# grero/HMMSpikeSorter.jl

Measured on AMD Instinct MI355X. Metric: Msamples/sec (Viterbi + forward-backward), K=4 L=60 HMM, higher is better.
Workload: dtype f64; 1 GPU; K=4 L=60 HMM (reference N=4, K=60: 237 states), 10000000-sample single channel per GPU: one Viterbi decode + one Baum-Welch E-step (forward-backward + sufficient statistics + M-step finish); channels=1, samples_per_channel=10000000, states=237, engine=wave, block=4928, halo=295, chains=2030, seed=1234, pooled_allreduce=False

## Files before the change

### hmmspikesorter.jl_amd/csrc/capi.cpp

```cpp
#include <algorithm>
#include <cstring>
#include <memory>

#include "hmmsort_internal.h"

using namespace hmmsort;

int hmmsort::need_device()
{
    int n = 0;
    hipError_t e = hipGetDeviceCount(&n);
    if (e != hipSuccess || n < 1) {
        (void)hipGetLastError();
        set_error("no HIP device available (%s); libhmmsort_hip has no CPU fallback",
                  e == hipSuccess ? "device count is 0" : hipGetErrorString(e));
        return HMMSORT_EHIP;
    }
    return HMMSORT_OK;
}

int hmmsort::plan_create_engine(hmmsort_plan **out, int64_t T, const int16_t *states, int64_t N, int64_t K,
                                int64_t S, const hmm_trans *tr, int64_t R, const double *mu, double sigma,
                                int64_t engine_req, int64_t halo_req)
{
    HS_CHECK(out, HMMSORT_EINVAL, "plan_create: null output pointer");
    *out = nullptr;
    HS_CHECK(T >= 1, HMMSORT_EINVAL, "plan_create: T must be >= 1 (got %lld)", (long long)T);
    int rc = need_device();
    if (rc) return rc;
    const Options opt = options_get();
    std::unique_ptr<hmmsort_plan> p(new hmmsort_plan());
    p->T = T;
    rc = build_host_model(p->model, states, N, K, S, tr, R, mu, sigma);
    if (rc) return rc;
    std::string why;
    const bool wave_ok = wave_supported(p->model, T, &why);
    if (engine_req == HMMSORT_ENGINE_WAVE && !wave_ok) {
        set_error("wave engine unavailable for this model/signal: %s", why.c_str());
        return HMMSORT_EUNSUP;
    }
    const bool ring_ok = ring_supported(p->model, T, &why);
    if (engine_req == HMMSORT_ENGINE_RING && !ring_ok) {
        set_error("ring engine unavailable for this model/signal: %s", why.c_str());
        return HMMSORT_EUNSUP;
    }
    const bool want_ring = engine_req == HMMSORT_ENGINE_RING;
    const int64_t halo = halo_req >= 0 ? halo_req : opt.halo;
    if ((engine_req == HMMSORT_ENGINE_AUTO || engine_req == HMMSORT_ENGINE_WAVE) && wave_ok) {
        p->models.assign(1, p->model);
        rc = wave_engine_create(&p->eng, p->models, T, opt.block, halo);
    } else if (want_ring && ring_ok) {
        rc = ring_engine_create(&p->eng, p->model, T, opt.block, halo);
    } else if (engine_req == HMMSORT_ENGINE_BLOCKED ||
               (engine_req == HMMSORT_ENGINE_AUTO && T >= blocked_min_samples())) {
        rc = generic_engine_create(&p->eng, p->model, T, true, opt.block, halo, opt.blocked_hbm_columns);
        if (rc == HMMSORT_EUNSUP && engine_req == HMMSORT_ENGINE_AUTO) rc = generic_engine_create(&p->eng, p->model, T);
    } else {
        rc = generic_engine_create(&p->eng, p->model, T);
    }
    if (rc) return rc;
    *out = p.release();
    return HMMSORT_OK;
}

extern "C" {

const char *hmmsort_last_error(void) { return last_error(); }
int hmmsort_version(void) { return 110;  }

int hmmsort_device_count(int *count)
{
    HS_CHECK(count, HMMSORT_EINVAL, "device_count: null pointer");
    int n = 0;
    if (hipGetDeviceCount(&n) != hipSuccess) {
        (void)hipGetLastError();
        n = 0;
    }
    *count = n;
    return HMMSORT_OK;
}

int hmmsort_set_device(int device)
{
    HS_HIP(hipSetDevice(device));
    return HMMSORT_OK;
}

int hmmsort_set_option(const char *key, int64_t value)
{
    HS_CHECK(key, HMMSORT_EINVAL, "set_option: null key");
    if (!strcmp(key, "engine")) {
        HS_CHECK(value >= 0 && value <= 4, HMMSORT_EINVAL, "set_option: engine must be 0..4");
        options_modify([&](Options &o) { o.engine = value; });
    } else if (!strcmp(key, "block")) {
        HS_CHECK(value >= 0, HMMSORT_EINVAL, "set_option: block must be >= 0");
        options_modify([&](Options &o) { o.block = value; });
    } else if (!strcmp(key, "halo")) {
        HS_CHECK(value >= 0, HMMSORT_EINVAL, "set_option: halo must be >= 0");
        options_modify([&](Options &o) { o.halo = value; });
    } else if (!strcmp(key, "escalate")) {
        options_modify([&](Options &o) { o.escalate = value != 0; });
    } else if (!strcmp(key, "strict_limit_mb")) {
        HS_CHECK(value >= 0, HMMSORT_EINVAL, "set_option: strict_limit_mb must be >= 0");
        options_modify([&](Options &o) { o.strict_limit_mb = value; });
    } else if (!strcmp(key, "blocked_hbm_columns")) {
        HS_CHECK(value >= 0 && value <= 2, HMMSORT_EINVAL, "set_option: blocked_hbm_columns must be 0..2");
        options_modify([&](Options &o) { o.blocked_hbm_columns = value; });
    } else if (!strcmp(key, "tie_scale")) {
        HS_CHECK(value >= 1, HMMSORT_EINVAL, "set_option: tie_scale must be >= 1");
        options_modify([&](Options &o) { o.tie_scale = value; });
    } else if (!strcmp(key, "tie_debug")) {
        HS_CHECK(value >= 0 && value <= 3, HMMSORT_EINVAL, "set_option: tie_debug must be 0..3");
        options_modify([&](Options &o) { o.tie_debug = value; });
    } else if (!strcmp(key, "backtrace")) {
        HS_CHECK(value >= 0 && value <= 2, HMMSORT_EINVAL, "set_option: backtrace must be 0..2");
        options_modify([&](Options &o) { o.backtrace = value; });
    } else if (!strcmp(key, "fit_streams")) {
        HS_CHECK(value >= 1 && value <= 16, HMMSORT_EINVAL, "set_option: fit_streams must be 1..16");
        options_modify([&](Options &o) { o.fit_streams = value; });
    } else if (!strcmp(key, "plan_cache")) {
        HS_CHECK(value >= 0 && value <= 64, HMMSORT_EINVAL, "set_option: plan_cache must be 0..64");
        options_modify([&](Options &o) { o.plan_cache = value; });
        host_slots_trim((size_t)value);
    } else {
        set_error("set_option: unknown key '%s'", key);
        return HMMSORT_EINVAL;
    }
    return HMMSORT_OK;
}

int hmmsort_get_option(const char *key, int64_t *value)
{
    HS_CHECK(key && value, HMMSORT_EINVAL, "get_option: null argument");
    const Options o = options_get();
    if (!strcmp(key, "engine")) *value = o.engine;
    else if (!strcmp(key, "block")) *value = o.block;
    else if (!strcmp(key, "halo")) *value = o.halo;
    else if (!strcmp(key, "escalate")) *value = o.escalate;
    else if (!strcmp(key, "plan_cache")) *value = o.plan_cache;
    else if (!strcmp(key, "strict_limit_mb")) *value = o.strict_limit_mb;
    else if (!strcmp(key, "blocked_hbm_columns")) *value = o.blocked_hbm_columns;
    else if (!strcmp(key, "tie_scale")) *value = o.tie_scale;
    else if (!strcmp(key, "tie_debug")) *value = o.tie_debug;
    else if (!strcmp(key, "backtrace")) *value = o.backtrace;
    else if (!strcmp(key, "fit_streams")) *value = o.fit_streams;
    else if (!strcmp(key, "last_escalations")) *value = last_escalations();
    else {
        set_error("get_option: unknown key '%s'", key);
        return HMMSORT_EINVAL;
    }
    return HMMSORT_OK;
}

int hmmsort_shutdown(void)
{
    host_slots_trim(0);
    return HMMSORT_OK;
}


int hmmsort_plan_create(hmmsort_plan **plan_out, int64_t T, const int16_t *states, int64_t N,
                        int64_t K, int64_t S, const hmm_trans *tr, int64_t R, const double *mu,
                        double sigma)
{
    return plan_create_engine(plan_out, T, states, N, K, S, tr, R, mu, sigma, options_get().engine);
}

int hmmsort_plan_create_batched(hmmsort_plan **plan_out, int64_t C, int64_t T, const int16_t *states,
                                int64_t N, int64_t K, int64_t S, const hmm_trans *tr, int64_t R,
                                const double *mu, const double *sigma)
{
    HS_CHECK(plan_out, HMMSORT_EINVAL, "plan_create_batched: null output pointer");
    *plan_out = nullptr;
    HS_CHECK(C >= 1 && C <= 4096 && T >= 1 && tr && mu && sigma, HMMSORT_EINVAL,
             "plan_create_batched: bad argument (C = %lld, T = %lld)", (long long)C, (long long)T);
    int rc = need_device();
    if (rc) return rc;
    std::unique_ptr<hmmsort_plan> p(new hmmsort_plan());
    p->T = T;
    p->C = C;
    p->models.resize(C);
    for (int64_t ch = 0; ch < C; ch++) {
        rc = build_host_model(p->models[ch], states, N, K, S, tr + ch * R, R, mu + ch * K * N, sigma[ch]);
        if (rc) return rc;
    }
    p->model = p->models[0];
    std::string why;
    if (!wave_supported(p->model, T, &why)) {
        set_error("plan_create_batched needs the wave engine: %s", why.c_str());
        return HMMSORT_EUNSUP;
    }
    const Options opt = options_get();
    rc = wave_engine_create(&p->eng, p->models, T, opt.block, opt.halo);
    if (rc) return rc;
    *plan_out = p.release();
    return HMMSORT_OK;
}

int64_t hmmsort_plan_channels(const hmmsort_plan *p) { return p ? p->C : 0; }

static int plan_set_model(const char *who, hmmsort_plan *p, int64_t channel, const hmm_trans *tr, int64_t R,
                          const double *mu, double sigma)
{
    HostModel m;
    std::vector<int16_t> st = p->model.states;
    int rc = build_host_model(m, st.data(), p->model.N, p->model.K, p->model.S, tr, R, mu, sigma);
    if (rc) return rc;
    HS_CHECK(!p->eng->ring_models_only() || m.ring.valid, HMMSORT_EUNSUP, "%s: new model is not a ring model", who);
    if ((rc = p->eng->set_model(channel, m))) return rc;
    if (!p->models.empty()) p->models[channel] = m;
    if (channel == 0) p->model = std::move(m);
    p->pu_stale = true;
    return HMMSORT_OK;
}

int hmmsort_plan_set_model_channel(hmmsort_plan *p, int64_t channel, const hmm_trans *tr, int64_t R,
                                   const double *mu, double sigma)
{
    HS_CHECK(p && tr && mu, HMMSORT_EINVAL, "plan_set_model_channel: null argument");
    HS_CHECK(p->eng->id == HMMSORT_ENGINE_WAVE, HMMSORT_EUNSUP, "plan_set_model_channel: needs a wave-engine plan");
    HS_CHECK(channel >= 0 && channel < p->C, HMMSORT_EINVAL, "plan_set_model_channel: channel %lld outside 0..%lld",
             (long long)channel, (long long)p->C - 1);
    return plan_set_model("plan_set_model_channel", p, channel, tr, R, mu, sigma);
}

int hmmsort_plan_set_model(hmmsort_plan *p, const hmm_trans *tr, int64_t R, const double *mu,
                           double sigma)
{
    HS_CHECK(p && tr && mu, HMMSORT_EINVAL, "plan_set_model: null argument");
    HS_CHECK(R == p->model.R || p->eng->ring_models_only(), HMMSORT_EINVAL,
             "plan_set_model: R changed (%lld -> %lld)", (long long)p->model.R, (long long)R);
    return plan_set_model("plan_set_model", p, 0, tr, R, mu, sigma);
}

int hmmsort_plan_destroy(hmmsort_plan *p)
{
    delete p;
    return HMMSORT_OK;
}

int hmmsort_plan_info(const hmmsort_plan *p, int64_t *engine, int64_t *block, int64_t *halo,
                      int64_t *nchains, int64_t *workspace_bytes)
{
    HS_CHECK(p, HMMSORT_EINVAL, "plan_info: null plan");
    int64_t b = 0, h = 0, n = 0;
    p->eng->geometry(&b, &h, &n);
    if (engine) *engine = p->eng->id;
    if (block) *block = b;
    if (halo) *halo = h;
    if (nchains) *nchains = n;
    if (workspace_bytes) *workspace_bytes = p->eng->workspace_bytes();
    return HMMSORT_OK;
}

int64_t hmmsort_plan_overlap_sweep(const hmmsort_plan *p) { return p ? p->eng->overlap_sweep() : 0; }

int hmmsort_plan_bind(hmmsort_plan *p, const double *d_y, void *stream)
{
    HS_CHECK(p && d_y, HMMSORT_EINVAL, "plan_bind: null argument");
    return p->eng->bind(d_y, (hipStream_t)stream);
}

int hmmsort_plan_unbind(hmmsort_plan *p)
{
    HS_CHECK(p, HMMSORT_EINVAL, "plan_unbind: null plan");
    p->eng->unbind();
    return HMMSORT_OK;
}

int hmmsort_plan_viterbi(hmmsort_plan *p, const double *d_y, int16_t *d_x, double *d_ll,
                         void *stream)
{
    HS_CHECK(p && d_y && d_x && d_ll, HMMSORT_EINVAL, "plan_viterbi: null argument");
    return p->eng->viterbi(d_y, d_x, d_ll, (hipStream_t)stream);
}

int hmmsort_plan_decode_estep(hmmsort_plan *p, const double *d_y, int16_t *d_x, double *d_ll,
                              double *d_stats, void *stream)
{
    HS_CHECK(p && d_y && d_x && d_ll && d_stats, HMMSORT_EINVAL, "plan_decode_estep: null argument");
    return p->eng->decode_estep(d_y, d_x, d_ll, d_stats, (hipStream_t)stream);
}

int hmmsort_plan_set_shard(hmmsort_plan *p, int64_t own_lo, int64_t own_hi, int first, int last)
{
    HS_CHECK(p, HMMSORT_EINVAL, "plan_set_shard: null plan");
    int rc = p->eng->set_shard(own_lo, own_hi, first != 0, last != 0);
    if (rc == HMMSORT_OK) p->sharded = !(own_lo == 0 && own_hi == p->T && first && last);
    return rc;
}

int64_t hmmsort_plan_stats_len(const hmmsort_plan *p) { return p ? p->eng->stats_len() : 0; }

int64_t hmmsort_plan_mstep_len(const hmmsort_plan *p)
{
    if (!p) return 0;
    const HostModel &m = p->model;
    return m.K * m.N + 1 + p->eng->n_lp() + m.S;
}

int hmmsort_plan_estep(hmmsort_plan *p, const double *d_y, double *d_stats, void *stream)
{
    HS_CHECK(p && d_y && d_stats, HMMSORT_EINVAL, "plan_estep: null argument");
    return p->eng->estep(d_y, d_stats, (hipStream_t)stream);
}

int hmmsort_plan_mstep(hmmsort_plan *p, const double *d_stats, double *d_out, void *stream)
{
    HS_CHECK(p && d_stats && d_out, HMMSORT_EINVAL, "plan_mstep: null argument");
    return p->eng->mstep(d_stats, d_out, (hipStream_t)stream);
}

int hmmsort_plan_path_update(hmmsort_plan *p, const double *d_y, const int16_t *d_x, double *d_out,
                             int64_t *d_counts, void *stream)
{
    HS_CHECK(p && d_y && d_x && d_out, HMMSORT_EINVAL, "plan_path_update: null argument");
    HS_CHECK(!p->sharded, HMMSORT_EINVAL, "plan_path_update: the plan is a time shard (hmmsort_plan_set_shard); the "
                                          "update needs the whole recording");
    return plan_path_update(p, d_y, d_x, d_out, d_counts, (hipStream_t)stream);
}

int hmmsort_plan_diagnostics(hmmsort_plan *p, void *stream, int64_t diag[8])
{
    HS_CHECK(p && diag, HMMSORT_EINVAL, "plan_diagnostics: null argument");
    for (int i = 0; i < 8; i++) diag[i] = 0;
    return p->eng->diagnostics((hipStream_t)stream, diag);
}

int hmmsort_plan_tie_stats(hmmsort_plan *p, void *stream, int64_t out[8])
{
    HS_CHECK(p && out, HMMSORT_EINVAL, "plan_tie_stats: null argument");
    for (int i = 0; i < 8; i++) out[i] = 0;
    return p->eng->tie_stats((hipStream_t)stream, out);
}

int hmmsort_plan_debug_record(hmmsort_plan *p, double *out64)
{
    HS_CHECK(p && out64, HMMSORT_EINVAL, "plan_debug_record: needs a wave plan");
    return p->eng->debug_record(out64);
}

int hmmsort_plan_debug_array(hmmsort_plan *p, int which, double *out, int64_t n)
{
    HS_CHECK(p && out, HMMSORT_EINVAL, "plan_debug_array: needs a wave plan");
    return p->eng->debug_array(which, out, n);
}

int hmmsort_plan_profile(hmmsort_plan *p, int enable)
{
    HS_CHECK(p, HMMSORT_EINVAL, "plan_profile: null plan");
    return p->eng->profile(enable);
}

int hmmsort_plan_profile_read(hmmsort_plan *p, void *stream, char *names, int64_t names_cap,
                              double *ms, int64_t *calls, int64_t cap, int64_t *n_out)
{
    HS_CHECK(p && names && ms && calls && n_out, HMMSORT_EINVAL, "plan_profile_read: null argument");
    *n_out = 0;
    if (names_cap > 0) names[0] = 0;
    std::vector<std::string> nm;
    std::vector<double> m;
    std::vector<int64_t> c;
    int rc = p->eng->profile_read((hipStream_t)stream, nm, m, c);
    if (rc) return rc;
    std::string joined;
    int64_t n = std::min<int64_t>((int64_t)nm.size(), cap);
    for (int64_t i = 0; i < n; i++) {
        if (i) joined += "\n";
        joined += nm[i];
        ms[i] = m[i];
        calls[i] = c[i];
    }
    HS_CHECK((int64_t)joined.size() + 1 <= names_cap, HMMSORT_EINVAL, "plan_profile_read: names buffer too small");
    memcpy(names, joined.c_str(), joined.size() + 1);
    *n_out = n;
    return HMMSORT_OK;
}

int hmmsort_samples_to_f64(const void *d_in, int sample_type, int64_t T, int64_t stride, double *d_out,
                           void *stream)
{
    HS_CHECK(T >= 0 && stride >= 1 && (T == 0 || (d_in && d_out)), HMMSORT_EINVAL,
             "samples_to_f64: bad argument (T = %lld, stride = %lld)", (long long)T, (long long)stride);
    int rc = need_device();
    if (rc) return rc;
    return dev_widen(d_in, sample_type, T, stride, d_out, (hipStream_t)stream);
}

int hmmsort_reconstruct(const int16_t *x, int64_t T, const int16_t *states, int64_t N, int64_t S,
                        const double *mu, int64_t K, double *y_out)
{
    HS_CHECK(states && mu && (T == 0 || (x && y_out)), HMMSORT_EINVAL, "reconstruct: null argument");
    HS_CHECK(T >= 0 && N >= 1 && S >= 1 && K >= 1, HMMSORT_EINVAL, "reconstruct: bad sizes");
    if (T == 0) return HMMSORT_OK;
    int rc = need_device();
    if (rc) return rc;
    for (int64_t i = 0; i < T; i++)
        HS_CHECK(x[i] >= 1 && x[i] <= S, HMMSORT_EINVAL,
                 "reconstruct: x[%lld] = %d outside 1..S (reference would throw BoundsError)",
                 (long long)i, (int)x[i]);
    DevBuf dx, dst, dmu, dout;
    if ((rc = dx.alloc(T * sizeof(int16_t))) || (rc = dst.alloc(N * S * sizeof(int16_t))) ||
        (rc = dmu.alloc(K * N * sizeof(double))) || (rc = dout.alloc(T * sizeof(double))))
        return rc;
    HS_HIP(hipMemcpy(dx.p, x, T * sizeof(int16_t), hipMemcpyHostToDevice));
    HS_HIP(hipMemcpy(dst.p, states, N * S * sizeof(int16_t), hipMemcpyHostToDevice));
    HS_HIP(hipMemcpy(dmu.p, mu, K * N * sizeof(double), hipMemcpyHostToDevice));
    rc = dev_reconstruct(dx.as<int16_t>(), T, dst.as<int16_t>(), N, S, dmu.as<double>(), K,
                         dout.as<double>(), nullptr);
    if (rc) return rc;
    HS_HIP(hipDeviceSynchronize());
    HS_HIP(hipMemcpy(y_out, dout.p, T * sizeof(double), hipMemcpyDeviceToHost));
    return HMMSORT_OK;
}

int hmmsort_unroll_mlseq(const int16_t *mlseq, int64_t T, const int16_t *states, int64_t N,
                         int64_t S, int16_t *out)
{
    HS_CHECK(states && (T == 0 || (mlseq && out)), HMMSORT_EINVAL, "unroll_mlseq: null argument");
    if (T == 0) return HMMSORT_OK;
    int rc = need_device();
    if (rc) return rc;
    for (int64_t i = 0; i < T; i++)
        HS_CHECK(mlseq[i] >= 1 && mlseq[i] <= S, HMMSORT_EINVAL,
                 "unroll_mlseq: mlseq[%lld] = %d outside 1..S", (long long)i, (int)mlseq[i]);
    DevBuf dx, dst, dout;
    if ((rc = dx.alloc(T * sizeof(int16_t))) || (rc = dst.alloc(N * S * sizeof(int16_t))) ||
        (rc = dout.alloc((size_t)N * T * sizeof(int16_t))))
        return rc;
    HS_HIP(hipMemcpy(dx.p, mlseq, T * sizeof(int16_t), hipMemcpyHostToDevice));
    HS_HIP(hipMemcpy(dst.p, states, N * S * sizeof(int16_t), hipMemcpyHostToDevice));
    rc = dev_unroll(dx.as<int16_t>(), T, dst.as<int16_t>(), N, S, dout.as<int16_t>(), nullptr);
    if (rc) return rc;
    HS_HIP(hipDeviceSynchronize());
    HS_HIP(hipMemcpy(out, dout.p, (size_t)N * T * sizeof(int16_t), hipMemcpyDeviceToHost));
    return HMMSORT_OK;
}

static int extract_from_device(const int16_t *d_x, int64_t T, const int16_t *states, int64_t N,
                               int64_t S, const double *mu, int64_t K, int64_t *times_out,
                               int64_t cap, int64_t *counts_out, hipStream_t st, DevBuf *dt_keep = nullptr)
{
    std::vector<uint32_t> match(S, 0u);
    for (int64_t i = 0; i < N; i++) {
        const int32_t qv = trough_value(mu, K, i);
        for (int64_t j = 0; j < S; j++)
// ... 153 lines not shown
```

### hmmspikesorter.jl_amd/csrc/hmmsort_internal.h

```cpp
#pragma once
#include <hip/hip_runtime.h>
#include <stdint.h>
#include <functional>
#include <memory>
#include <string>
#include <vector>
#include "../../include/hmmsort.h"

namespace hmmsort {

void set_error(const char *fmt, ...);
const char *last_error();

#define HS_HIP(call)                                                                          \
    do {                                                                                      \
        hipError_t e_ = (call);                                                               \
        if (e_ != hipSuccess) {                                                               \
            hmmsort::set_error("%s failed: %s (%s:%d)", #call, hipGetErrorString(e_),         \
                               __FILE__, __LINE__);                                           \
            return HMMSORT_EHIP;                                                              \
        }                                                                                     \
    } while (0)

#define HS_CHECK(cond, code, ...)                                                             \
    do {                                                                                      \
        if (!(cond)) {                                                                        \
            hmmsort::set_error(__VA_ARGS__);                                                  \
            return (code);                                                                    \
        }                                                                                     \
    } while (0)

constexpr double kLog2Pi = 0.9189385332046727;

struct Options {
    int64_t engine = HMMSORT_ENGINE_AUTO;
    int64_t block = 0;
    int64_t halo = 0;
    int64_t escalate = 1;
    int64_t plan_cache = 4;
    int64_t strict_limit_mb = 0;
    int64_t tie_scale = 1;
    int64_t blocked_hbm_columns = 0;
    int64_t tie_debug = 0;
    int64_t fit_streams = 4;
    int64_t backtrace = 0;
};
Options options_get();
void options_modify(const std::function<void(Options &)> &f);
int64_t &last_escalations();

struct RingModel {
    bool valid = false;
    int N = 0, L = 0;
    double c00 = 0;
    std::vector<double> c0;
    std::vector<double> cint;
    std::vector<double> cend;
    std::vector<double> cx;
};

struct HostModel {
    int64_t N = 0, K = 0, S = 0, R = 0;
    std::vector<int16_t> states;
    std::vector<hmm_trans> tr;
    std::vector<double> mu;
    double sigma = 0;
    std::vector<double> mean;
    std::vector<int32_t> in_ptr, in_src;
    std::vector<double> in_lp;
    std::vector<int32_t> out_ptr, out_dst;
    std::vector<double> out_lp;
    RingModel ring;
};

int build_host_model(HostModel &m, const int16_t *states, int64_t N, int64_t K, int64_t S,
                     const hmm_trans *tr, int64_t R, const double *mu, double sigma);
int analyze_ring(const HostModel &m, RingModel &ring);
inline int32_t trough_value(const double *mu, int64_t K, int64_t i)
{
    int64_t q = 0;
    for (int64_t k = 1; k < K; k++)
        if (mu[k + K * i] < mu[q + K * i]) q = k;
    return (int32_t)(q + 1);
}
inline double strict_limit_bytes(const Options &opt)
{
    size_t free_b = 0, total_b = 0;
    if (hipMemGetInfo(&free_b, &total_b) != hipSuccess) { (void)hipGetLastError(); free_b = 0; }
    return opt.strict_limit_mb > 0 ? (double)opt.strict_limit_mb * 1048576.0 : 0.9 * (double)free_b;
}

struct DevBuf {
    void *p = nullptr;
    size_t cap = 0;
    ~DevBuf() { release(); }
    void release()
    {
        if (p) (void)hipFree(p);
        p = nullptr;
        cap = 0;
    }
    int alloc(size_t bytes)
    {
        release();
        bytes = bytes < 8 ? 8 : bytes;
        if (hipMalloc(&p, bytes) != hipSuccess) {
            (void)hipGetLastError();
            set_error("hipMalloc of %zu bytes failed", bytes);
            p = nullptr;
            return HMMSORT_ENOMEM;
        }
        cap = bytes;
        return HMMSORT_OK;
    }
    int ensure(size_t bytes) { return (p && cap >= (bytes < 8 ? 8 : bytes)) ? HMMSORT_OK : alloc(bytes); }
    template <typename Tv> Tv *as() { return static_cast<Tv *>(p); }
};

class Engine {
public:
    const int64_t id;
    explicit Engine(int64_t id_) : id(id_) {}
    virtual ~Engine() = default;
    Engine(const Engine &) = delete;
    Engine &operator=(const Engine &) = delete;

    virtual int set_model(int64_t channel, const HostModel &m) = 0;
    virtual bool ring_models_only() const { return false; }
    virtual void geometry(int64_t *block, int64_t *halo, int64_t *nchains) const = 0;
    virtual int64_t workspace_bytes() const = 0;
    virtual int bind(const double *, hipStream_t) { return HMMSORT_OK; }
    virtual void unbind() {}
    virtual int viterbi(const double *d_y, int16_t *d_x, double *d_ll, hipStream_t st) = 0;
    virtual int decode_estep(const double *, int16_t *, double *, double *, hipStream_t)
    {
        return refuse(HMMSORT_EUNSUP, "plan_decode_estep: needs the wave or ring engine");
    }
    virtual int64_t stats_len() const { return 0; }
    bool has_estep() const { return stats_len() > 0; }
    virtual int estep(const double *, double *, hipStream_t)
    {
        return refuse(HMMSORT_EUNSUP, "plan_estep: sufficient-statistics E-step needs the wave, ring or blocked "
                                      "engine (use hmmsort_em_step)");
    }
    virtual int mstep(const double *, double *, hipStream_t)
    {
        return refuse(HMMSORT_EUNSUP, "plan_mstep: needs the wave, ring or blocked engine");
    }
    virtual int64_t n_lp() const = 0;
    virtual int set_shard(int64_t, int64_t, bool, bool)
    {
        return refuse(HMMSORT_EUNSUP, "plan_set_shard: needs the wave or ring engine");
    }
    virtual int diagnostics(hipStream_t, int64_t[8]) { return HMMSORT_OK; }
    virtual int tie_stats(hipStream_t, int64_t[8]) { return HMMSORT_OK; }
    virtual int profile(int) { return HMMSORT_OK; }
    virtual int profile_read(hipStream_t, std::vector<std::string> &, std::vector<double> &, std::vector<int64_t> &)
    {
        return HMMSORT_OK;
    }
    virtual bool has_posteriors() const { return false; }
    virtual int posteriors(const HostModel &, const double *, double *, double *, double *, double *, hipStream_t)
    {
        set_error("plan_posteriors: needs a wave plan (ring models), a blocked plan (overlap models within the LDS "
                  "limit) or a strict plan (any model); this plan runs engine %lld", (long long)id);
        return HMMSORT_EUNSUP;
    }
    virtual bool posteriors_valid() const { return false; }
    virtual int posterior_decode(int16_t *, hipStream_t)
    {
        return refuse(HMMSORT_EINVAL, "plan_posterior_decode: call hmmsort_plan_posteriors first");
    }
    virtual int spike_conf(int, int, int, int64_t, const int64_t *, int64_t, double *, hipStream_t)
    {
        return refuse(HMMSORT_EINVAL, "plan_spike_confidence: call hmmsort_plan_posteriors first");
    }
    virtual int expected_counts(double *, hipStream_t)
    {
        return refuse(HMMSORT_EINVAL, "plan_expected_counts: call hmmsort_plan_posteriors first");
    }
    virtual int64_t overlap_sweep() const { return 0; }
    virtual bool drop_structured_sweep() { return false; }
    virtual int forward(const double *, double *, hipStream_t) { return refuse(HMMSORT_EUNSUP, "forward: needs the strict engine"); }
    virtual int backward(const double *, double *, hipStream_t) { return refuse(HMMSORT_EUNSUP, "backward: needs the strict engine"); }
    virtual int update(const double *, const double *, const double *, double *, hipStream_t)
    {
        return refuse(HMMSORT_EUNSUP, "update: needs the strict engine");
    }
    virtual int debug_record(double *) { return refuse(HMMSORT_EINVAL, "plan_debug_record: needs a wave plan"); }
    virtual int debug_array(int, double *, int64_t) { return refuse(HMMSORT_EINVAL, "plan_debug_array: needs a wave plan"); }

protected:
    static int refuse(int code, const char *msg)
    {
        set_error("%s", msg);
        return code;
    }
    static int check_shard(int64_t T, int64_t own_lo, int64_t own_hi, bool first, bool last)
    {
        HS_CHECK(own_lo >= 0 && own_lo <= own_hi && own_hi <= T, HMMSORT_EINVAL,
                 "plan_set_shard: owned range [%lld, %lld) outside [0, %lld]", (long long)own_lo,
                 (long long)own_hi, (long long)T);
        HS_CHECK((!first || own_lo == 0) && (!last || own_hi == T), HMMSORT_EINVAL,
                 "plan_set_shard: a first/last shard must own its first/last sample");
        return HMMSORT_OK;
    }
};

bool wave_supported(const HostModel &m, int64_t T, std::string *why);
int wave_engine_create(std::unique_ptr<Engine> *out, const std::vector<HostModel> &models, int64_t T,
                       int64_t block_req, int64_t halo_req);
int ring_engine_create(std::unique_ptr<Engine> *out, const HostModel &m, int64_t T, int64_t block_req,
                       int64_t halo_req);
int generic_engine_create(std::unique_ptr<Engine> *out, const HostModel &m, int64_t T, bool blocked = false,
                          int64_t block_req = 0, int64_t halo_req = 0, int64_t hbm_columns = 0);

struct GenericDev;
struct RingDev;
struct PathUpdateDev;

int generic_create(GenericDev **g, const HostModel &m, int64_t T, bool blocked = false,
                   int64_t block_req = 0, int64_t halo_req = 0);
bool generic_pair_active(const GenericDev *g);
void generic_pair_disable(GenericDev *g);
int64_t generic_overlap_sweep(const GenericDev *g);
int64_t blocked_min_samples();
int generic_set_model(GenericDev *g, const HostModel &m);
void generic_destroy(GenericDev *g);
int generic_viterbi(GenericDev *g, const double *d_y, int16_t *d_x, double *d_ll,
                    hipStream_t st);
int generic_forward(GenericDev *g, const double *d_y, double *d_alpha, hipStream_t st);
int generic_backward(GenericDev *g, const double *d_y, double *d_beta, hipStream_t st);
int generic_update(GenericDev *g, const double *d_alpha, const double *d_beta, const double *d_y,
                   double *d_out, hipStream_t st);
int generic_posteriors(const double *d_alpha, const double *d_beta, int64_t T, int64_t S, int64_t N,
                       const int16_t *d_states, const int32_t *d_qv, double *d_logz, double *d_onset,
                       double *d_occ, double *d_silent, double *d_tq, int16_t *d_xm, hipStream_t st);
bool blocked_estep_supported(const GenericDev *g);
void blocked_set_hbm_columns(GenericDev *g, int64_t v);
bool blocked_post_supported(const GenericDev *g);
int blocked_posteriors(GenericDev *g, const double *d_y, const int32_t *trough, double *d_onset, double *d_occ,
                       double *d_silent, double *d_tq, int16_t *d_xm, double *d_logz, hipStream_t st);

int ring_create(RingDev **r, const HostModel &m, int64_t T, int64_t block_req, int64_t halo_req);
int ring_set_model(RingDev *r, const HostModel &m);
void ring_destroy(RingDev *r);
int ring_diagnostics(RingDev *r, hipStream_t st, int64_t diag[8]);
bool ring_supported(const HostModel &m, int64_t T, std::string *why);

int dev_reconstruct(const int16_t *d_x, int64_t T, const int16_t *d_states, int64_t N, int64_t S,
                    const double *d_mu, int64_t K, double *d_out, hipStream_t st);
int dev_widen(const void *d_in, int dtype, int64_t T, int64_t stride, double *d_out, hipStream_t st);
constexpr int kSpikeChunkHost = 4096;
int dev_spike_compact(const int16_t *d_x, int64_t T, const uint32_t *d_match, int N, int S, int pass,
                      int64_t *d_cnt, const int64_t *d_offs, int64_t *d_times, int64_t cap,
                      hipStream_t st);
int dev_unroll(const int16_t *d_x, int64_t T, const int16_t *d_states, int64_t N, int64_t S,
               int16_t *d_out, hipStream_t st);
int dev_chunk_stitch(const int16_t *d_x, int64_t k, bool lead, bool trail, int16_t *d_dst, int64_t *d_lk,
                     hipStream_t st);
int dev_fill_i16(int16_t *d_p, int64_t n, int16_t v, hipStream_t st);
int dev_chunk_ll(const double *d_y, const int16_t *d_x, int64_t k, int64_t S, const double *d_mean,
                 const int32_t *d_in_ptr, const int32_t *d_in_src, const double *d_in_lp, double sigma, double *d_pv,
                 double *d_ll, hipStream_t st);
constexpr int kPostParts = 256;
int dev_spike_conf(const double *d_src, const double *d_head, int64_t T, int64_t shift, int64_t jitter,
                   const int64_t *d_times, int64_t n, double *d_conf, hipStream_t st);
int dev_row_sums(const double *d_rows, int64_t nrows, int64_t T, double *d_part, double *out_host, hipStream_t st);

}

struct hmmsort_plan {
    hmmsort::HostModel model;
    std::vector<hmmsort::HostModel> models;
    int64_t T = 0;
    int64_t C = 1;
    std::unique_ptr<hmmsort::Engine> eng;
    bool sharded = false;
    std::shared_ptr<hmmsort::PathUpdateDev> pu;
    bool pu_stale = true;
};

namespace hmmsort {
int need_device();
int plan_create_engine(hmmsort_plan **out, int64_t T, const int16_t *states, int64_t N, int64_t K, int64_t S,
                       const hmm_trans *tr, int64_t R, const double *mu, double sigma, int64_t engine_req,
                       int64_t halo_req = -1);
struct PlanGuard {
    hmmsort_plan *p = nullptr;
    ~PlanGuard() { if (p) hmmsort_plan_destroy(p); }
};
int plan_path_update(hmmsort_plan *p, const double *d_y, const int16_t *d_x, double *d_out, int64_t *d_counts,
                     hipStream_t st);
void host_slots_trim(size_t keep);
}
```

### hmmspikesorter.jl_amd/csrc/wave_common.h

```cpp
#pragma once
#include <hip/hip_runtime.h>
#include <stdint.h>
#include <cmath>
#include <cstring>
#include <string>
#include <vector>

#include "hmmsort_internal.h"
#include "ring_common.h"

namespace hmmsort {

constexpr double kScFloor = -700.0;

struct WaveGeom {
    int64_t T;
    int C;
    int N, L;
    int W;
    int RB;
    int B;
    int Hw;
    int He;
    int nch;
    int EB, epw, PW;
    int Bb, Hb;
    int64_t nseg;
    int64_t own_lo, own_hi;
    int first, last;
    double thr_scale;
    int tie_debug;
    int backtrace;
};

struct WaveConst {
    double c00, mean0, den, A, sc0, P00;
    double c0[kRingMaxN], cend[kRingMaxN], sc[kRingMaxN], CP0[kRingMaxN], PEND[kRingMaxN];
    double xishift[kRingMaxN];
    double cx[kRingMaxN * kRingMaxN];
    double CPX[kRingMaxN * kRingMaxN];
    double cxin[kRingMaxN];
    double CPXin[kRingMaxN];
    double cxT[kRingMaxN * kRingMaxN];
    double CPXT[kRingMaxN * kRingMaxN];
};

struct WaveDev {
    WaveGeom g{};
    bool prof_on = false;
    bool uniform_cx = true;
    std::vector<char> ucx;
    const double *bound_y = nullptr;
    hipStream_t side = nullptr, side2 = nullptr;
    hipEvent_t ev_fork = nullptr, ev_join = nullptr, ev_a = nullptr, ev_b = nullptr, ev_c = nullptr, ev_x = nullptr;
    std::vector<ProfEntry> prof;
    int64_t S = 0, K = 0;
    std::vector<RingModel> ring;
    std::vector<std::vector<double>> mean;
    std::vector<double> sigma;
    WaveConst *d_cst = nullptr;
    double *d_mean = nullptr;
    double *d_meanT = nullptr;
    double *d_msq = nullptr;
    double *d_cint = nullptr;
    double *d_ctab = nullptr;
    int16_t *d_states = nullptr;
    double *Rf = nullptr;
    double *W2 = nullptr;
    double *virt = nullptr;
    double *ysum = nullptr;
    uint32_t *psi = nullptr;
    double *vpre = nullptr, *vend = nullptr;
    int32_t *vfail = nullptr;
    int32_t *bstate = nullptr;
    int32_t *redo = nullptr;
    int32_t *final_state = nullptr;
    double *part = nullptr;
    double *FA0 = nullptr;
    double *FV = nullptr;
    double *FREF = nullptr;
    double *fpre = nullptr;
    double *bpre = nullptr, *bown = nullptr;
    double *rho = nullptr;
    double *Zc = nullptr;
    double *partS = nullptr;
    double *partG = nullptr;
    double *yhead = nullptr;
    double *extra = nullptr;
    double *pp = nullptr;
    int64_t *diag = nullptr;
    int32_t *heads = nullptr;
    int32_t *vlist = nullptr;
    double *trash = nullptr;
    double *dbg = nullptr;
    bool keep_post = false;
    bool post_valid = false;
    double *gsil = nullptr;
    double *phead = nullptr;
    double *plogz = nullptr;
    double *pcnt = nullptr;
    int64_t *tie_cnt = nullptr;
    int64_t *tie_list = nullptr;
    int64_t *tie_off = nullptr;
    int64_t tie_ntile = 0;
    int16_t *tie_walk = nullptr;
    double *tie_guess = nullptr;
    double *tie_c = nullptr;
    int32_t *tie_ok = nullptr;
    double *tie_v = nullptr;
    int64_t tie_nblk = 0;
    struct GraphEntry { uint64_t key[12]; hipGraphExec_t exec; };
    std::vector<GraphEntry> graphs;
    bool graphs_on = true;
    int64_t bytes = 0;
    int nparts = 0, gparts = 0;
};

struct WProfScope {
    WaveDev *r;
    hipStream_t st;
    ProfEntry e;
    WProfScope(WaveDev *r_, const char *name, hipStream_t st_) : r(r_), st(st_)
    {
        e.name = name; e.a = nullptr; e.b = nullptr;
        if (r->prof_on && hipEventCreate(&e.a) == hipSuccess && hipEventCreate(&e.b) == hipSuccess)
            (void)hipEventRecord(e.a, st);
    }
    ~WProfScope()
    {
        if (r->prof_on && e.a && e.b) {
            (void)hipEventRecord(e.b, st);
            r->prof.push_back(e);
        }
    }
};
#define WPROF(r, name, st) WProfScope wprof_scope_(r, name, st)

constexpr int wpsi_bits_c(int N) { int b = 1; while ((1 << b) < N + 1) b++; return b + 1; }
constexpr int wpsi_epw_c(int N) { return 32 / wpsi_bits_c(N); }
constexpr int wpsi_words_c(int N) { return (N + 1 + wpsi_epw_c(N) - 1) / wpsi_epw_c(N); }

__device__ __forceinline__ double wave_bcast(double v, int lane)
{
    const int lo = __builtin_amdgcn_readlane(__double2loint(v), lane);
    const int hi = __builtin_amdgcn_readlane(__double2hiint(v), lane);
    return __hiloint2double(hi, lo);
}

template <int CTRL, int ROWMASK>
__device__ __forceinline__ double dpp_mov(double old, double v)
{
    const int lo = __builtin_amdgcn_update_dpp(__double2loint(old), __double2loint(v), CTRL, ROWMASK, 0xF, false);
    const int hi = __builtin_amdgcn_update_dpp(__double2hiint(old), __double2hiint(v), CTRL, ROWMASK, 0xF, false);
    return __hiloint2double(hi, lo);
}

__device__ __forceinline__ double lane_prev(double v, double carry)
{
    return dpp_mov<0x138, 0xF>(carry, v);
}

__device__ __forceinline__ void scan_maxplus(double &a, double &b)
{
#define HS_MP_STEP(CTRL, RM)                                                      \
    {                                                                             \
        const double al = dpp_mov<CTRL, RM>(0.0, a), bl = dpp_mov<CTRL, RM>(-INFINITY, b); \
        b = fmax(bl + a, b);                                                      \
        a = al + a;                                                               \
    }
    HS_MP_STEP(0x111, 0xF) HS_MP_STEP(0x112, 0xF) HS_MP_STEP(0x114, 0xF) HS_MP_STEP(0x118, 0xF)
    HS_MP_STEP(0x142, 0xA) HS_MP_STEP(0x143, 0xC)
#undef HS_MP_STEP
}

template <int CTRL, int ROWMASK>
__device__ __forceinline__ float dpp_movf(float old, float v)
{
    return __int_as_float(__builtin_amdgcn_update_dpp(__float_as_int(old), __float_as_int(v), CTRL, ROWMASK, 0xF, false));
}
__device__ __forceinline__ void scan_maxplus_f32(float &a, float &b)
{
#define HS_MPF_STEP(CTRL, RM)                                                     \
    {                                                                             \
        const float al = dpp_movf<CTRL, RM>(0.0f, a), bl = dpp_movf<CTRL, RM>(-INFINITY, b); \
        b = fmaxf(bl + a, b);                                                     \
        a = al + a;                                                               \
    }
    HS_MPF_STEP(0x111, 0xF) HS_MPF_STEP(0x112, 0xF) HS_MPF_STEP(0x114, 0xF) HS_MPF_STEP(0x118, 0xF)
    HS_MPF_STEP(0x142, 0xA) HS_MPF_STEP(0x143, 0xC)
#undef HS_MPF_STEP
}
__device__ __forceinline__ float lane_prevf(float v, float carry)
{
    return dpp_movf<0x138, 0xF>(carry, v);
}

__device__ __forceinline__ void scan_linear(double &a, double &b)
{
#define HS_LN_STEP(CTRL, RM)                                                      \
    {                                                                             \
        const double al = dpp_mov<CTRL, RM>(1.0, a), bl = dpp_mov<CTRL, RM>(0.0, b); \
        b = __builtin_fma(a, bl, b);                                              \
        a = al * a;                                                               \
    }
    HS_LN_STEP(0x111, 0xF) HS_LN_STEP(0x112, 0xF) HS_LN_STEP(0x114, 0xF) HS_LN_STEP(0x118, 0xF)
    HS_LN_STEP(0x142, 0xA) HS_LN_STEP(0x143, 0xC)
#undef HS_LN_STEP
}

__device__ __forceinline__ double lane_prev_ref(double v, double carry, int lane)
{
    const double s = __shfl_up(v, 1);
    return lane == 0 ? carry : s;
}
__device__ __forceinline__ void scan_maxplus_ref(double &a, double &b, int lane)
{
#pragma unroll
    for (int d = 1; d < 64; d <<= 1) {
        const double al = __shfl_up(a, d), bl = __shfl_up(b, d);
        if (lane >= d) { b = fmax(bl + a, b); a = al + a; }
    }
}
__device__ __forceinline__ void scan_linear_ref(double &a, double &b, int lane)
{
#pragma unroll
    for (int d = 1; d < 64; d <<= 1) {
        const double al = __shfl_up(a, d), bl = __shfl_up(b, d);
        if (lane >= d) { b = __builtin_fma(a, bl, b); a = al * a; }
    }
}

__device__ __forceinline__ const WaveConst *reload_consts(const WaveConst *p)
{
    asm volatile("" : "+s"(p));
    return p;
}

template <int N> constexpr int wave_depth() { return N <= 4 ? 4 : (N <= 8 ? 3 : 2); }
template <int N> constexpr int wave_occ() { return N <= 4 ? 4 : (N <= 8 ? 2 : 1); }

__device__ __forceinline__ double wave_max(double v)
{
#pragma unroll
    for (int o = 32; o > 0; o >>= 1) v = fmax(v, __shfl_xor(v, o));
    return v;
}
__device__ __forceinline__ double wave_sum(double v)
{
#pragma unroll
    for (int o = 32; o > 0; o >>= 1) v += __shfl_xor(v, o);
    return v;
}

__device__ __forceinline__ void wave_lds_order()
{
    __builtin_amdgcn_fence(__ATOMIC_RELEASE, "wavefront");
    __builtin_amdgcn_wave_barrier();
    __builtin_amdgcn_fence(__ATOMIC_ACQUIRE, "wavefront");
}

constexpr int kTieBlk = 512;
constexpr int kTieCap = 65536;
constexpr int kTieWalk = 8192;
constexpr int kTieLanes = 64;
constexpr int kTieTrig = 0;
constexpr int kTieListed = 1;
constexpr int kTieDone = 2;
constexpr int kTieFlips = 3;
constexpr int kTieOpen = 4;
constexpr int kTieTail = 5;
constexpr int kTieLongest = 6;
constexpr int kTieSerial = 7;

__device__ __forceinline__ double wpath_lp(int N, int L, const double *__restrict__ ctab, int xp, int xc)
{
    if (xp == 1) return xc == 1 ? ctab[0] : ctab[1 + (xc - 2) / L];
    const int a = (xp - 2) / L, k = (xp - 2) % L + 1;
    if (k < L) return ctab[1 + 2 * N + N * N + a * L + k];
    if (xc == 1) return ctab[1 + N + a];
    return ctab[1 + 2 * N + a * N + (xc - 2) / L];
}

__device__ __forceinline__ double wave_thr(const WaveGeom &g, const WaveConst &K, const double *__restrict__ ysum, int ch)
{
    const double T = (double)g.T;
    const double s1 = ysum[2 * ch], s2 = ysum[2 * ch + 1];
    const double sq = fmax((s2 - 2.0 * K.mean0 * s1) + T * K.mean0 * K.mean0, 0.0);
    const double mmax = fabs(K.A) * T + sq / K.den + fabs(K.c00) * T + 1.0;
    return (ldexp(16.0 * (double)(g.L + 2), ilogb(mmax) - 52) + 4.0e-9) * g.thr_scale;
}

template <typename F>
int wave_graphed(WaveDev *r, int kind, const void *p0, const void *p1, const void *p2, const void *p3,
                 hipStream_t st, F enqueue)
{
    if (!r->graphs_on || r->prof_on || st == nullptr) return enqueue(st);
    uint64_t key[12] = {(uint64_t)kind, (uint64_t)(uintptr_t)p0, (uint64_t)(uintptr_t)p1, (uint64_t)(uintptr_t)p2,
                        (uint64_t)(uintptr_t)p3, (uint64_t)(uintptr_t)st, (uint64_t)(r->bound_y == p0),
                        (uint64_t)r->uniform_cx, (uint64_t)r->g.own_lo, (uint64_t)r->g.own_hi,
                        (uint64_t)(r->g.first * 2 + r->g.last), (uint64_t)(uint32_t)r->g.tie_debug};
    {
        uint64_t tb;
        static_assert(sizeof(tb) == sizeof(r->g.thr_scale), "");
        memcpy(&tb, &r->g.thr_scale, sizeof(tb));
        key[11] ^= tb << 8;
    }
    for (auto &e : r->graphs)
        if (!memcmp(e.key, key, sizeof(key))) {
            HS_HIP(hipGraphLaunch(e.exec, st));
            return HMMSORT_OK;
        }
    if (hipStreamBeginCapture(st, hipStreamCaptureModeRelaxed) != hipSuccess) {
        (void)hipGetLastError();
        r->graphs_on = false;
        return enqueue(st);
    }
    const int rc = enqueue(st);
    hipGraph_t graph = nullptr;
    const hipError_t e1 = hipStreamEndCapture(st, &graph);
    hipGraphExec_t exec = nullptr;
    if (rc || e1 != hipSuccess || !graph || hipGraphInstantiate(&exec, graph, nullptr, nullptr, 0) != hipSuccess) {
        (void)hipGetLastError();
        if (graph) (void)hipGraphDestroy(graph);
        r->graphs_on = false;
        return rc ? rc : enqueue(st);
    }
    (void)hipGraphDestroy(graph);
    if (r->graphs.size() >= 16) {
        (void)hipGraphExecDestroy(r->graphs.front().exec);
        r->graphs.erase(r->graphs.begin());
    }
    WaveDev::GraphEntry ge;
    memcpy(ge.key, key, sizeof(key));
    ge.exec = exec;
    r->graphs.push_back(ge);
    HS_HIP(hipGraphLaunch(exec, st));
    return HMMSORT_OK;
}

inline size_t wave_zero_bytes(const WaveDev *r, bool decode)
{
    return (size_t)(decode ? 8 + 8 * (int64_t)r->g.C + 2 : 8) * sizeof(int64_t);
}

int wave_create(WaveDev **out, const std::vector<HostModel> &models, int64_t T, int64_t block_req,
                int64_t halo_req);
int wave_set_model(WaveDev *r, int ch, const HostModel &m);
void wave_destroy(WaveDev *r);
int wave_prepare(WaveDev *r, const double *d_y, hipStream_t st);
int wave_bind(WaveDev *r, const double *d_y, hipStream_t st);
int64_t wave_stats_len(const WaveDev *r);
int wave_diagnostics(WaveDev *r, hipStream_t st, int64_t diag[8]);
int wave_profile_read(WaveDev *r, hipStream_t st, std::vector<std::string> &names,
                      std::vector<double> &ms, std::vector<int64_t> &calls);
int wave_viterbi_sweep(WaveDev *r, const double *d_y, hipStream_t st);
int wave_viterbi_post(WaveDev *r, const double *d_y, int16_t *d_x, double *d_ll, hipStream_t st, bool beside,
                      bool ll_beside, hipStream_t ll_st);
int wave_viterbi(WaveDev *r, const double *d_y, int16_t *d_x, double *d_ll, hipStream_t st);
int wave_tie_resolve(WaveDev *r, const double *d_y, int16_t *d_x, hipStream_t st);
int wave_tie_stats(WaveDev *r, hipStream_t st, int64_t out[8]);
int wave_estep(WaveDev *r, const double *d_y, double *d_stats, hipStream_t st);
int wave_mstep(WaveDev *r, const double *d_stats, double *d_out, hipStream_t st);
int wave_decode_estep(WaveDev *r, const double *d_y, int16_t *d_x, double *d_ll, double *d_stats,
                      hipStream_t st);
int wave_post_sweeps(WaveDev *r, const double *d_y, hipStream_t st);
int wave_posteriors(WaveDev *r, const double *d_y, double *d_onset, double *d_occ, double *d_silent, double *d_logz,
                    hipStream_t st);
int wave_post_decode(WaveDev *r, int16_t *d_xm, hipStream_t st);
int wave_spike_conf(WaveDev *r, int ch, int a, int qv, int64_t jitter, const int64_t *d_times, int64_t n,
                    double *d_conf, hipStream_t st);
int wave_expected_counts(WaveDev *r, double *counts_out, hipStream_t st);

}
```

### hmmspikesorter.jl_amd/csrc/wave_engine.hip

```cpp
#include <algorithm>
#include <cmath>
#include <cstdlib>
#include <cstring>
#include <type_traits>

#include "wave_common.h"

namespace hmmsort {

static inline int64_t wround_up(int64_t v, int64_t m) { return (v + m - 1) / m * m; }

constexpr int64_t kWaveLdsMax = 160 * 1024;

static bool ring_uniform_cx(const RingModel &R)
{
    const int N = R.N;
    for (int a = 0; a < N; a++) {
        double ref = 0.0;
        bool have = false;
        for (int b = 0; b < N; b++) {
            if (b == a) continue;
            const double v = R.cx[b * N + a];
            if (!have) { ref = v; have = true; }
            else if (!(v == ref)) return false;
        }
    }
    return true;
}

constexpr int kWaveMaxPerSource = 8;

bool wave_supported(const HostModel &m, int64_t T, std::string *why)
{
    auto no = [&](const char *w) { if (why) *why = w; return false; };
    if (!m.ring.valid) return no("transition list is not the no-overlap ring pattern");
    if (m.ring.N > kRingMaxN) return no("more than 16 rings");
    if (m.ring.N > kWaveMaxPerSource && !ring_uniform_cx(m.ring))
        return no("exit->entry log-probabilities depend on the source ring and there are more than 8 rings");
    if (m.ring.L < 8) return no("rings shorter than 8 states");
    if (T < 4 * (int64_t)m.ring.L || T < 512) return no("signal shorter than 4 ring lengths / 512 samples");
    const int W = std::min(m.ring.L, 64);
    const int64_t RB = wround_up(m.ring.L + W, 32);
    const int64_t lines = m.ring.N > 8 ? m.ring.N + 1 : 2 * (int64_t)m.ring.N;
    if (lines * (RB + 1) * 8 + 4096 > kWaveLdsMax) return no("delay lines exceed the LDS of one CU");
    return true;
}

static int make_geometry(WaveGeom &g, int64_t T, int C, int N, int L, int64_t block_req, int64_t halo_req)
{
    g.T = T; g.C = C; g.N = N; g.L = L;
    g.own_lo = 0; g.own_hi = T; g.first = 1; g.last = 1;
    { const Options o = options_get(); g.thr_scale = (double)o.tie_scale; g.tie_debug = (int)o.tie_debug;
      g.backtrace = (int)o.backtrace; }
    g.W = std::min(L, 64);
    g.RB = (int)wround_up(L + g.W, 32);
    int64_t H = halo_req > 0 ? halo_req : std::max<int64_t>(256, 4 * (int64_t)L);
    H = std::max<int64_t>(H, L + 8);
    const int64_t m = (H + g.W - 1) / g.W;
    g.Hw = (int)(1 + m * g.W);
    g.He = (int)(m * g.W);
    int64_t B = block_req > 0 ? block_req : (T * C + 2047) / 2048;
    B = std::max<int64_t>(B, std::max<int64_t>(2 * g.Hw, 512));
    if (block_req > 0) B = std::max<int64_t>(block_req, std::max<int64_t>(g.Hw, L + 16));
    B = wround_up(B, 64);
    if (B > T) B = wround_up(T, 64);
    for (;;) {
        const int64_t nch = (T + B - 1) / B;
        const int64_t nlast = T - (nch - 1) * B;
        if (nch == 1 || nlast >= L) break;
        B += 64;
    }
    HS_CHECK(B < (1 << 30), HMMSORT_EINVAL, "wave engine: chain too long");
    g.B = (int)B;
    g.nch = (int)((T + B - 1) / B);
    int bits = 1;
    while ((1 << bits) < N + 1) bits++;
    g.EB = bits + 1; g.epw = 32 / g.EB; g.PW = (N + 1 + g.epw - 1) / g.epw;
    g.Bb = 512; g.Hb = 128;
    while (g.Hb < 2 * L + 64) g.Hb += 64;
    if (g.Bb < 2 * g.Hb) g.Bb = 2 * g.Hb;
    g.nseg = (T + g.Bb - 1) / g.Bb;
    return HMMSORT_OK;
}

template <typename Tv>
static int wmalloc(Tv **p, int64_t n, int64_t *bytes)
{
    if (hipMalloc((void **)p, (size_t)std::max<int64_t>(n, 1) * sizeof(Tv)) != hipSuccess) {
        (void)hipGetLastError();
        set_error("wave engine: hipMalloc of %.2f GB failed", n * sizeof(Tv) / 1e9);
        *p = nullptr;
        return HMMSORT_ENOMEM;
    }
    *bytes += n * (int64_t)sizeof(Tv);
    return HMMSORT_OK;
}

int wave_set_model(WaveDev *r, int ch, const HostModel &m)
{
    const WaveGeom &g = r->g;
    HS_CHECK(ch >= 0 && ch < g.C, HMMSORT_EINVAL, "wave set_model: channel %d outside 0..%d", ch, g.C - 1);
    HS_CHECK(m.ring.valid && m.ring.N == g.N && m.ring.L == g.L && m.S == r->S, HMMSORT_EINVAL,
             "wave set_model: model shape changed");
    HS_CHECK(g.N <= kWaveMaxPerSource || ring_uniform_cx(m.ring), HMMSORT_EUNSUP,
             "wave set_model: exit->entry log-probabilities depend on the source ring and there are more than 8 rings");
    r->bound_y = nullptr;
    r->ring[ch] = m.ring;
    r->mean[ch] = m.mean;
    r->sigma[ch] = m.sigma;
    const int N = g.N, L = g.L;
    const RingModel &R = m.ring;
    WaveConst k;
    memset(&k, 0, sizeof(k));
    k.c00 = R.c00;
    k.mean0 = m.mean[0];
    k.den = 2.0 * (m.sigma * m.sigma);
    k.A = -kLog2Pi - std::log(m.sigma);
    double sc0 = R.c00;
    for (int a = 0; a < N; a++) sc0 = std::max(sc0, R.cend[a]);
    if (!std::isfinite(sc0)) sc0 = 0.0;
    k.sc0 = sc0;
    k.P00 = std::exp(R.c00 - sc0);
    for (int a = 0; a < N; a++) {
        k.c0[a] = R.c0[a];
        k.cend[a] = R.cend[a];
        k.PEND[a] = std::exp(R.cend[a] - sc0);
        double sc = R.c0[a];
        for (int b = 0; b < N; b++)
            if (b != a) sc = std::max(sc, R.cx[b * N + a]);
        if (!std::isfinite(sc)) sc = 0.0;
        sc = std::max(sc, kScFloor);
        k.sc[a] = sc;
        k.CP0[a] = std::exp(R.c0[a] - sc);
        k.xishift[a] = R.c0[a] - sc;
    }
    for (int a = 0; a < N; a++)
        for (int b = 0; b < N; b++) {
            k.cx[a * N + b] = (a == b) ? -INFINITY : R.cx[a * N + b];
            k.CPX[a * N + b] = (a == b) ? 0.0 : std::exp(R.cx[a * N + b] - k.sc[b]);
            k.cxT[b * N + a] = k.cx[a * N + b];
            k.CPXT[b * N + a] = k.CPX[a * N + b];
        }
    bool ucx = true;
    for (int a = 0; a < N; a++) {
        double ref = -INFINITY;
        bool have = false;
        for (int b = 0; b < N; b++) {
            if (b == a) continue;
            const double v = R.cx[b * N + a];
            if (!have) { ref = v; have = true; }
            else if (!(v == ref)) ucx = false;
        }
        k.cxin[a] = have ? ref : -INFINITY;
        k.CPXin[a] = have ? std::exp(ref - k.sc[a]) : 0.0;
    }
    r->ucx[ch] = ucx;
    r->uniform_cx = true;
    for (char u : r->ucx) r->uniform_cx = r->uniform_cx && u;
    HS_HIP(hipMemcpy(r->d_cst + ch, &k, sizeof(k), hipMemcpyHostToDevice));
    HS_HIP(hipMemcpy(r->d_mean + (size_t)ch * m.S, m.mean.data(), m.S * sizeof(double), hipMemcpyHostToDevice));
    {
        const int Nn = m.ring.N, Ll = m.ring.L;
        std::vector<double> mt((size_t)Nn * Ll);
        for (int a = 0; a < Nn; a++)
            for (int k = 0; k < Ll; k++) mt[(size_t)k * Nn + a] = m.mean[1 + (size_t)a * Ll + k];
        HS_HIP(hipMemcpy(r->d_meanT + (size_t)ch * Nn * Ll, mt.data(), mt.size() * sizeof(double), hipMemcpyHostToDevice));
    }
    std::vector<double> cint((size_t)N * (L + 1), 0.0), msq((size_t)N * (L + 1), 0.0);
    for (int a = 0; a < N; a++) {
        double acc = 0.0, acc2 = 0.0;
        for (int kk = 2; kk <= L; kk++) {
            acc += R.cint[(size_t)a * L + (kk - 1)];
            cint[(size_t)a * (L + 1) + kk] = acc;
        }
        for (int kk = 1; kk <= L; kk++) {
            const double mv = m.mean[1 + (size_t)a * L + (kk - 1)];
            acc2 += mv * mv;
            msq[(size_t)a * (L + 1) + kk] = acc2;
        }
    }
    const size_t nt = (size_t)N * (L + 1);
    HS_HIP(hipMemcpy(r->d_cint + ch * nt, cint.data(), nt * sizeof(double), hipMemcpyHostToDevice));
    HS_HIP(hipMemcpy(r->d_msq + ch * nt, msq.data(), nt * sizeof(double), hipMemcpyHostToDevice));
    std::vector<double> ctab;
    ctab.push_back(R.c00);
    ctab.insert(ctab.end(), R.c0.begin(), R.c0.end());
    ctab.insert(ctab.end(), R.cend.begin(), R.cend.end());
    ctab.insert(ctab.end(), R.cx.begin(), R.cx.end());
    ctab.insert(ctab.end(), R.cint.begin(), R.cint.end());
    HS_HIP(hipMemcpy(r->d_ctab + (size_t)ch * ctab.size(), ctab.data(), ctab.size() * sizeof(double),
                     hipMemcpyHostToDevice));
    if (ch == 0)
        HS_HIP(hipMemcpy(r->d_states, m.states.data(), m.states.size() * sizeof(int16_t), hipMemcpyHostToDevice));
    return HMMSORT_OK;
}

int wave_create(WaveDev **out, const std::vector<HostModel> &models, int64_t T, int64_t block_req,
                int64_t halo_req)
{
    HS_CHECK(!models.empty(), HMMSORT_EINVAL, "wave engine: no model");
    const HostModel &m = models[0];
    std::string why;
    HS_CHECK(wave_supported(m, T, &why), HMMSORT_EUNSUP, "wave engine: %s", why.c_str());
    const int C = (int)models.size();
    WaveDev *r = new WaveDev();
    int rc = make_geometry(r->g, T, C, m.ring.N, m.ring.L, block_req, halo_req);
    if (rc) { delete r; return rc; }
    r->S = m.S; r->K = m.K;
    r->graphs_on = getenv("HMMSORT_GRAPHS") && atoi(getenv("HMMSORT_GRAPHS")) != 0;
    r->ring.resize(C); r->mean.resize(C); r->sigma.resize(C); r->ucx.assign(C, 1);
    const WaveGeom &g = r->g;
    const int64_t N = g.N, L = g.L, CT = (int64_t)C * T, nchT = (int64_t)C * g.nch;
    r->nparts = 1024;
    bool ok = true;
    auto A = [&](auto **p, int64_t n) { if (ok && wmalloc(p, n, &r->bytes)) ok = false; };
    A(&r->d_cst, C);
    A(&r->d_mean, C * m.S);
    A(&r->d_meanT, C * N * L);
    A(&r->d_cint, C * N * (L + 1));
    A(&r->d_msq, C * N * (L + 1));
    A(&r->d_ctab, C * (1 + 2 * N + N * N + N * L));
    A(&r->d_states, N * m.S);
    A(&r->Rf, N * CT);
    A(&r->W2, CT);
    A(&r->virt, C * N * (L + 1));
    A(&r->ysum, 2 * C);
    A(&r->psi, (int64_t)g.PW * CT);
    A(&r->vpre, nchT * (1 + N * L));
    A(&r->vend, nchT * (1 + N * L));
    A(&r->vfail, nchT + 8);
    A(&r->bstate, C * g.nseg);
    A(&r->redo, 2 * C * g.nseg + 8);
    A(&r->vlist, 2 * nchT + 8);
    A(&r->final_state, C + 8);
    A(&r->part, (int64_t)C * 4 * r->nparts);
    A(&r->FA0, CT);
    A(&r->FV, N * CT);
    A(&r->FREF, CT);
    A(&r->fpre, nchT * (1 + L * (N + 1)));
    A(&r->bpre, nchT * (1 + L * (N + 1)));
    A(&r->bown, nchT * (1 + L * (N + 1)));
    A(&r->rho, N * CT);
    A(&r->Zc, nchT);
    A(&r->partS, nchT * (3 * N + 3));
    r->gparts = (int)((T + 4095) / 4096);
    r->gparts = std::max<int>(r->gparts, g.nch);
    A(&r->partG, (int64_t)C * r->gparts * N * L);
    A(&r->yhead, C * (N * L + 2));
    A(&r->extra, C * 3 * N * L);
    A(&r->pp, C * m.S);
    A(&r->diag, 8 + 8 * (int64_t)C + 2);
    if (ok) { r->tie_cnt = r->diag + 8; r->heads = reinterpret_cast<int32_t *>(r->diag + 8 + 8 * (int64_t)C); }
    A(&r->dbg, 64);
    A(&r->trash, 64 * 64);
    r->tie_nblk = (T + kTieBlk - 1) / kTieBlk;
    A(&r->tie_list, (int64_t)C * kTieCap);
    r->tie_ntile = (T + 4095) / 4096;
    A(&r->tie_off, (int64_t)C * (r->tie_ntile + 1));
    A(&r->tie_walk, (int64_t)C * kTieLanes * kTieWalk);
    A(&r->tie_guess, (int64_t)C * r->tie_nblk);
    A(&r->tie_c, (int64_t)C * r->tie_nblk * 2);
    A(&r->tie_ok, (int64_t)C * r->tie_nblk);
    A(&r->tie_v, (int64_t)C * (r->tie_nblk + 1));
    if (!ok) { wave_destroy(r); return HMMSORT_ENOMEM; }
    if (getenv("HMMSORT_POISON")) {
        (void)hipMemset(r->Rf, 0xFF, N * CT * 8);
        (void)hipMemset(r->psi, 0xFF, (int64_t)g.PW * CT * 4);
        (void)hipMemset(r->vpre, 0xFF, nchT * (1 + N * L) * 8);
        (void)hipMemset(r->vend, 0xFF, nchT * (1 + N * L) * 8);
        (void)hipMemset(r->FA0, 0xFF, CT * 8);
        (void)hipMemset(r->FV, 0xFF, N * CT * 8);
        (void)hipMemset(r->FREF, 0xFF, CT * 8);
        (void)hipMemset(r->fpre, 0xFF, nchT * (1 + L * (N + 1)) * 8);
        (void)hipMemset(r->bpre, 0xFF, nchT * (1 + L * (N + 1)) * 8);
        (void)hipMemset(r->bown, 0xFF, nchT * (1 + L * (N + 1)) * 8);
        (void)hipMemset(r->rho, 0xFF, N * CT * 8);
        (void)hipMemset(r->Zc, 0xFF, nchT * 8);
        (void)hipMemset(r->partS, 0xFF, nchT * (3 * N + 3) * 8);
        (void)hipMemset(r->partG, 0xFF, (int64_t)C * r->gparts * N * L * 8);
        (void)hipMemset(r->yhead, 0xFF, C * (N * L + 2) * 8);
    }
    if (hipMemset(r->diag, 0, wave_zero_bytes(r, true)) != hipSuccess ||
        hipMemset(r->vfail, 0, (nchT + 8) * sizeof(int32_t)) != hipSuccess) {
        wave_destroy(r);
        return HMMSORT_EHIP;
    }
    for (int ch = 0; ch < C; ch++) {
        const HostModel &mc = models[ch];
        if (mc.S != m.S || mc.K != m.K || mc.N != m.N) {
            set_error("wave engine: channel %d has a different model shape", ch);
            wave_destroy(r);
            return HMMSORT_EINVAL;
        }
        rc = wave_set_model(r, ch, mc);
        if (rc) { wave_destroy(r); return rc; }
    }
    if (hipStreamCreateWithFlags(&r->side, hipStreamNonBlocking) != hipSuccess ||
        hipStreamCreateWithFlags(&r->side2, hipStreamNonBlocking) != hipSuccess ||
        hipEventCreateWithFlags(&r->ev_fork, hipEventDisableTiming) != hipSuccess ||
        hipEventCreateWithFlags(&r->ev_join, hipEventDisableTiming) != hipSuccess ||
        hipEventCreateWithFlags(&r->ev_a, hipEventDisableTiming) != hipSuccess ||
        hipEventCreateWithFlags(&r->ev_b, hipEventDisableTiming) != hipSuccess ||
        hipEventCreateWithFlags(&r->ev_c, hipEventDisableTiming) != hipSuccess ||
        hipEventCreateWithFlags(&r->ev_x, hipEventDisableTiming) != hipSuccess) {
        set_error("wave engine: could not create the internal stream/events");
        wave_destroy(r);
        return HMMSORT_EHIP;
    }
    *out = r;
    return HMMSORT_OK;
}

void wave_destroy(WaveDev *r)
{
    if (!r) return;
    void *ptrs[] = {r->d_cst, r->d_mean, r->d_meanT, r->d_cint, r->d_msq, r->d_ctab, r->d_states, r->Rf, r->W2, r->virt, r->ysum,
                    r->psi, r->vpre, r->vend, r->vfail, r->bstate, r->redo, r->final_state, r->part, r->FA0,
                    r->FV, r->FREF, r->fpre, r->bpre, r->bown, r->rho, r->Zc, r->partS, r->partG, r->yhead,
                    r->extra, r->pp, r->diag, r->vlist, r->dbg, r->trash, r->tie_list, r->tie_off, r->tie_walk, r->tie_guess,
                    r->tie_c, r->tie_ok, r->tie_v, r->gsil, r->phead, r->plogz, r->pcnt};
    for (void *p : ptrs)
        if (p) (void)hipFree(p);
    if (r->ev_fork) (void)hipEventDestroy(r->ev_fork);
    if (r->ev_join) (void)hipEventDestroy(r->ev_join);
    if (r->ev_a) (void)hipEventDestroy(r->ev_a);
    if (r->ev_b) (void)hipEventDestroy(r->ev_b);
    if (r->ev_c) (void)hipEventDestroy(r->ev_c);
    if (r->ev_x) (void)hipEventDestroy(r->ev_x);
    if (r->side) (void)hipStreamDestroy(r->side);
    if (r->side2) (void)hipStreamDestroy(r->side2);
    for (auto &e : r->prof) { (void)hipEventDestroy(e.a); (void)hipEventDestroy(e.b); }
    for (auto &ge : r->graphs) (void)hipGraphExecDestroy(ge.exec);
    delete r;
}

int wave_diagnostics(WaveDev *r, hipStream_t st, int64_t diag[8])
{
    HS_HIP(hipStreamSynchronize(st));
    HS_HIP(hipMemcpy(diag, r->diag, 8 * sizeof(int64_t), hipMemcpyDeviceToHost));
    return HMMSORT_OK;
}

int64_t wave_stats_len(const WaveDev *r) { return 3 * (int64_t)r->g.N * r->g.L + r->g.N + 4; }

__device__ __forceinline__ void virtual_onsets(const WaveGeom &g, int ch, const WaveConst *__restrict__ cst,
                                               const double *__restrict__ y, const double *__restrict__ mean,
                                               const double *__restrict__ cint, double *__restrict__ virt)
{
    const int L = g.L, N = g.N, S = 1 + N * L;
    const double *yc = y + (int64_t)ch * g.T, *mc = mean + (int64_t)ch * S;
    const double *ci = cint + (int64_t)ch * N * (L + 1);
    const double den = cst[ch].den, A = cst[ch].A;
    for (int i = threadIdx.x; i < N * L; i += blockDim.x) {
        const int a = i / L, j = i % L + 1;
        double v;
        if (j == L) {
            v = -INFINITY;
        } else if (j == L - 1) {
            const double d = yc[0] - mc[1 + a * L + (L - 1)];
            v = (A - (d * d) / den) - A;
        } else {
            double acc = 0.0;
            for (int k0 = 1 + j; k0 <= L; k0 += 8) {
                double yv[8], mv[8];
#pragma unroll
                for (int u = 0; u < 8; u++) {
                    const int k = k0 + u <= L ? k0 + u : L;
                    yv[u] = yc[k - 1 - j]; mv[u] = mc[1 + a * L + (k - 1)];
                }
#pragma unroll
                for (int u = 0; u < 8; u++) {
                    const double d = yv[u] - mv[u];
                    if (k0 + u <= L) acc += d * d;
                }
            }
            v = (ci[a * (L + 1) + L] - ci[a * (L + 1) + (1 + j)]) - acc / den;
        }
        virt[((int64_t)ch * N + a) * (L + 1) + j] = v;
    }
}

template <int N> constexpr int pre_rows() { return N <= 4 ? 8 : 4; }

template <int N> static size_t pre_lds(int L)
{
    constexpr int R = pre_rows<N>();
    const int n = 256 * R + (L > 256 ? L : 256);
    return (size_t)(n + n / R + 2) * sizeof(double);
}

template <int N>
__global__ __launch_bounds__(256) void kw_prepass(WaveGeom g, const WaveConst *__restrict__ cst,
                                                  const double *__restrict__ y,
                                                  const double *__restrict__ mean,
                                                  const double *__restrict__ cint,
                                                  const double *__restrict__ msq,
                                                  double *__restrict__ Rf, double *__restrict__ W2,
                                                  double *__restrict__ ysum, const double *__restrict__ mean_states,
                                                  double *__restrict__ virt)
{
    constexpr int R = pre_rows<N>(), TILE = 256 * R;
    extern __shared__ double ly[];
    __shared__ double red[8];
    const int ch = blockIdx.y, L = g.L, tid = threadIdx.x;
    if (blockIdx.x == 0) {
        virtual_onsets(g, ch, cst, y, mean_states, cint, virt);
        return;
    }
    const int64_t T = g.T, t0 = (int64_t)(blockIdx.x - 1) * TILE;
    const double *yc = y + (int64_t)ch * T;
    const double *mc = mean + (int64_t)ch * N * L;
    auto pad = [](int i) { return i + i / R; };
    double s1 = 0.0, s2 = 0.0;
    {
        const double *yt = yc + t0;
        const int nv = (int)(T - t0 < TILE + 512 ? T - t0 : TILE + 512);
        double v[R + 1];
#pragma unroll
        for (int q = 0; q <= R; q++) {
            const unsigned i = tid + 256 * q;
            v[q] = yt[i < (unsigned)nv ? i : (unsigned)nv - 1u];
        }
#pragma unroll
        for (int q = 0; q <= R; q++) {
            const int i = tid + 256 * q;
            const double yv = i < nv ? v[q] : 0.0;
            ly[pad(i)] = yv;
            if (q < R) { s1 += yv; s2 = __builtin_fma(yv, yv, s2); }
        }
        for (int i = TILE + 256 + tid; i < TILE + L; i += 256) {
            const int64_t t = t0 + i;
            const double yv = yc[t < T ? t : T - 1];
            ly[pad(i)] = t < T ? yv : 0.0;
        }
    }
    s1 = wave_sum(s1); s2 = wave_sum(s2);
    if ((tid & 63) == 0) { red[tid >> 6] = s1; red[4 + (tid >> 6)] = s2; }
    __syncthreads();
    if (tid == 0) {
        atomicAdd(&ysum[2 * ch], (red[0] + red[1]) + (red[2] + red[3]));
        atomicAdd(&ysum[2 * ch + 1], (red[4] + red[5]) + (red[6] + red[7]));
    }
    constexpr int U = R + 1;
    double dot[R][N], ysq[R], w[U];
#pragma unroll
    for (int r = 0; r < R; r++) {
        ysq[r] = 0.0;
        w[r] = ly[pad(R * tid + r)];
#pragma unroll
        for (int a = 0; a < N; a++) dot[r][a] = 0.0;
    }
    double mv[N];
#pragma unroll
    for (int a = 0; a < N; a++) mv[a] = mc[a];
    for (int k0 = 0; k0 < L; k0 += U) {
#pragma unroll
        for (int kk = 0; kk < U; kk++) {
            const int k = k0 + kk;
            if (k < L) {
                const int kn = k + 1 < L ? k + 1 : k;
                double mn[N];
#pragma unroll
                for (int a = 0; a < N; a++) mn[a] = mc[kn * N + a];
                w[(kk + R) % U] = ly[pad(R * tid + k + R)];
#pragma unroll
                for (int r = 0; r < R; r++) {
                    const double yv = w[(r + kk) % U];
                    ysq[r] = __builtin_fma(yv, yv, ysq[r]);
#pragma unroll
                    for (int a = 0; a < N; a++) dot[r][a] = __builtin_fma(yv, mv[a], dot[r][a]);
                }
#pragma unroll
                for (int a = 0; a < N; a++) mv[a] = mn[a];
            }
        }
    }
    const double rden = 1.0 / cst[ch].den;
    const bool interior = t0 + TILE + L <= T;
    auto value = [&](int a, int r, double msqL, double cintL, int64_t cb) {
        double mq = msqL, ci = cintL;
        if (!interior) {
            const int64_t rem = T - (t0 + R * tid + r);
            const int kmax = rem < L ? (rem > 0 ? (int)rem : 0) : L;
            mq = msq[cb + kmax]; ci = cint[cb + kmax];
        }
        return ci - ((ysq[r] - 2.0 * dot[r][a]) + mq) * rden;
    };
    {
        __syncthreads();
        const int lane = tid & 63, seg = (tid >> 6) * (64 * R);
#pragma unroll
        for (int a = 0; a <= N; a++) {
            const int64_t cb = ((int64_t)ch * N + (a < N ? a : 0)) * (L + 1);
            const double msqL = msq[cb + L], cintL = cint[cb + L];
            wave_lds_order();
#pragma unroll
            for (int r = 0; r < R; r++)
                ly[pad(R * tid + r)] = a < N ? value(a < N ? a : 0, r, msqL, cintL, cb) : ysq[r];
            wave_lds_order();
            double *dst = a < N ? Rf + ((int64_t)ch * N + a) * T : W2 + (int64_t)ch * T;
#pragma unroll
            for (int q = 0; q < R; q++) {
                const int i = seg + lane + 64 * q;
                const double o = ly[pad(i)];
                if (t0 + i < T) dst[t0 + i] = o;
            }
        }
    }
}

int wave_prepare(WaveDev *r, const double *d_y, hipStream_t st)
{
    if (r->bound_y == d_y) return HMMSORT_OK;
    r->bound_y = nullptr;
    const WaveGeom &g = r->g;
    HS_HIP(hipMemsetAsync(r->ysum, 0, 2 * g.C * sizeof(double), st));
    int rc = dispatch_N(g.N, [&](auto n) {
        constexpr int N = decltype(n)::value;
        WPROF(r, "kw_prepass", st);
        constexpr int kPreTile = 256 * pre_rows<N>();
        hipLaunchKernelGGL((kw_prepass<N>), dim3(1 + (unsigned)((g.T + kPreTile - 1) / kPreTile), g.C), dim3(256),
                           pre_lds<N>(g.L), st, g, r->d_cst, d_y, r->d_meanT, r->d_cint,
                           r->d_msq, r->Rf, r->W2, r->ysum, r->d_mean, r->virt);
        HS_HIP(hipGetLastError());
        return HMMSORT_OK;
    });
    return rc;
}

int wave_bind(WaveDev *r, const double *d_y, hipStream_t st)
{
    r->bound_y = nullptr;
    int rc = wave_prepare(r, d_y, st);
    if (rc) return rc;
    r->bound_y = d_y;
    return HMMSORT_OK;
}

int wave_profile_read(WaveDev *r, hipStream_t st, std::vector<std::string> &names,
                      std::vector<double> &ms, std::vector<int64_t> &calls)
{
    HS_HIP(hipStreamSynchronize(st));
    if (r->side) HS_HIP(hipStreamSynchronize(r->side));
    if (r->side2) HS_HIP(hipStreamSynchronize(r->side2));
    for (auto &e : r->prof) {
        float t = 0.f;
        if (hipEventElapsedTime(&t, e.a, e.b) != hipSuccess) { (void)hipGetLastError(); t = 0.f; }
        size_t i = 0;
        for (; i < names.size(); i++)
            if (names[i] == e.name) break;
        if (i == names.size()) { names.push_back(e.name); ms.push_back(0.0); calls.push_back(0); }
        ms[i] += t;
        calls[i] += 1;
        (void)hipEventDestroy(e.a);
        (void)hipEventDestroy(e.b);
    }
    r->prof.clear();
    return HMMSORT_OK;
}

namespace {
struct WaveEngine final : Engine {
    WaveDev *w = nullptr;
    WaveEngine() : Engine(HMMSORT_ENGINE_WAVE) {}
    ~WaveEngine() override { wave_destroy(w); }
    int set_model(int64_t ch, const HostModel &m) override { return wave_set_model(w, (int)ch, m); }
    bool ring_models_only() const override { return true; }
    void geometry(int64_t *b, int64_t *h, int64_t *n) const override
    {
        *b = w->g.B; *h = w->g.Hw - 1; *n = (int64_t)w->g.nch * w->g.C;
    }
    int64_t workspace_bytes() const override { return w->bytes; }
    int bind(const double *d_y, hipStream_t st) override { return wave_bind(w, d_y, st); }
    void unbind() override { w->bound_y = nullptr; }
    int viterbi(const double *d_y, int16_t *d_x, double *d_ll, hipStream_t st) override
    {
        return wave_viterbi(w, d_y, d_x, d_ll, st);
    }
    int decode_estep(const double *d_y, int16_t *d_x, double *d_ll, double *d_stats, hipStream_t st) override
    {
        return wave_decode_estep(w, d_y, d_x, d_ll, d_stats, st);
    }
    int64_t stats_len() const override { return wave_stats_len(w); }
    int estep(const double *d_y, double *d_stats, hipStream_t st) override { return wave_estep(w, d_y, d_stats, st); }
    int mstep(const double *d_stats, double *d_out, hipStream_t st) override { return wave_mstep(w, d_stats, d_out, st); }
    int64_t n_lp() const override { return w->g.N; }
    int set_shard(int64_t own_lo, int64_t own_hi, bool first, bool last) override
    {
        WaveGeom &g = w->g;
        if (int rc = check_shard(g.T, own_lo, own_hi, first, last)) return rc;
        const int64_t B = g.B, last_boundary = (int64_t)(g.nch - 1) * B;
        HS_CHECK(first || (g.nch > 1 && own_lo >= B), HMMSORT_EINVAL,
                 "plan_set_shard: no chain boundary inside the leading halo (owned range starts at %lld, chains are "
                 "%lld samples): widen the halo or set a shorter chain length (option \"block\")",
                 (long long)own_lo, (long long)B);
        HS_CHECK(last || (g.nch > 1 && own_hi <= last_boundary), HMMSORT_EINVAL,
                 "plan_set_shard: no chain boundary inside the trailing halo (owned range ends at %lld, last chain "
                 "boundary at %lld): widen the halo or set a shorter chain length (option \"block\")",
                 (long long)own_hi, (long long)last_boundary);
        g.own_lo = own_lo; g.own_hi = own_hi;
        g.first = first; g.last = last;
        return HMMSORT_OK;
    }
    int diagnostics(hipStream_t st, int64_t diag[8]) override { return wave_diagnostics(w, st, diag); }
    int tie_stats(hipStream_t st, int64_t out[8]) override { return wave_tie_stats(w, st, out); }
    int profile(int enable) override { w->prof_on = enable != 0; return HMMSORT_OK; }
    int profile_read(hipStream_t st, std::vector<std::string> &names, std::vector<double> &ms,
                     std::vector<int64_t> &calls) override
    {
        return wave_profile_read(w, st, names, ms, calls);
    }
    bool has_posteriors() const override { return true; }
    int posteriors(const HostModel &, const double *d_y, double *d_onset, double *d_occ, double *d_silent,
                   double *d_logz, hipStream_t st) override
    {
        return wave_posteriors(w, d_y, d_onset, d_occ, d_silent, d_logz, st);
    }
    bool posteriors_valid() const override { return w->post_valid; }
    int posterior_decode(int16_t *d_xm, hipStream_t st) override { return wave_post_decode(w, d_xm, st); }
    int spike_conf(int ch, int a, int qv, int64_t jitter, const int64_t *d_times, int64_t n, double *d_conf,
                   hipStream_t st) override
    {
        return wave_spike_conf(w, ch, a, qv, jitter, d_times, n, d_conf, st);
    }
    int expected_counts(double *counts_out, hipStream_t st) override { return wave_expected_counts(w, counts_out, st); }
    int debug_record(double *out64) override
    {
        HS_HIP(hipDeviceSynchronize());
        HS_HIP(hipMemcpy(out64, w->dbg, 64 * sizeof(double), hipMemcpyDeviceToHost));
        return HMMSORT_OK;
    }
// ... 64 lines not shown
```

### hmmspikesorter.jl_amd/csrc/wave_estep.hip

```cpp
#include <cmath>
#include <type_traits>

#include "fastmath.h"
#include "wave_common.h"

namespace hmmsort {

constexpr double kLn2 = 6.93147180559945286227e-01;
typedef double wg_d4 __attribute__((ext_vector_type(4)));

__device__ __forceinline__ double scale_of(double v, double s)
{
    return v > 0.0 ? s + (double)ilogb(v) * kLn2 : -INFINITY;
}

template <int N>
struct FIn {
    double y;
    double R[N];
};

template <int N>
__device__ __forceinline__ void excl_sums(const double (&t)[N], double (&out)[N])
{
// ... 791 lines not shown
            const int a = i % NP, u = (i / NP) % RRL, cc = i / (NP * RRL);
            if (u < RR) lr[cc * RS + (u + u / 16) * NP + a] = tr_[k];
        }
#pragma unroll
        for (int k = 0; k < NYM; k++) {
            const int i = tid + k * 256;
            const int rr = i % YRL, cc = i / YRL;
            if (rr < YR - 1) ly[cc * YR + rr] = ty_[k];
        }
        __syncthreads();
        if (ti + 1 < ntiles) load_regs(ti + 1);
#pragma unroll
        for (int h = 0; h < CW / 4; h++) {
            const int cc = wv * (CW / 4) + h;
            const double *lyc = ly + cc * YR + lk + lj;
#pragma unroll 4
            for (int ts = 0; ts < TR / 4; ts++) {
                const int u = lk - 16 * lsft + HS + 4 * ts;
                const double b = lr[cc * RS + (u + u / 16) * NP + la];
#pragma unroll
                for (int q = 0; q < NT; q++) {
                    const double a = lyc[ts * 4 + q * LPT];
                    c1[q] = __builtin_amdgcn_mfma_f64_16x16x4f64(a, b, c1[q], 0, 0, 0);
                }
            }
        }
    }
    const int NL = N * L;
    double *out = partG + ((int64_t)ch * nparts + blockIdx.x) * NL;
    double *red = lds;
#pragma unroll
    for (int q = 0; q < NT; q++) {
        __syncthreads();
#pragma unroll
        for (int r = 0; r < 4; r++) red[(wv * 4 + r) * 64 + lane] = c1[q][r];
        __syncthreads();
        {
            const int e = tid;
            const int ln = e & 63, r = e >> 6;
            double v = 0.0;
#pragma unroll
            for (int w = 0; w < 4; w++) v += red[(w * 4 + r) * 64 + ln];
            const int j = ln & 15, a = j % NP, sft = j / NP;
            const int lag = lag0 + q * LPT + 16 * sft + (ln >> 4) + 4 * r;
            if (a < N && lag < L) out[a * L + lag] = v;
        }
    }
}

__global__ __launch_bounds__(64) void kw_stats_final(WaveGeom g, int rowsG, const double *__restrict__ partG,
                                                     const double *__restrict__ partS, const double *__restrict__ y,
                                                     const double *__restrict__ Rf, const double *__restrict__ virt,
                                                     const double *__restrict__ FA0, const double *__restrict__ rho,
                                                     const double *__restrict__ Zc, const double *__restrict__ yhead,
                                                     double *__restrict__ pp, double *__restrict__ stats)
{
    const int N = g.N, L = g.L, i = blockIdx.x, ch = blockIdx.y, lane = threadIdx.x;
    const int NL = N * L, ws = 3 * N + 3, total = 3 * NL + N + 4, S = 1 + NL;
    const double *pS = partS + (int64_t)ch * g.nch * ws;
    const double *pG = partG + (int64_t)ch * rowsG * NL;
    auto colsum = [&](const double *p, int rows, size_t stride) {
        double a0 = 0.0, a1 = 0.0, a2 = 0.0, a3 = 0.0, a4 = 0.0, a5 = 0.0, a6 = 0.0, a7 = 0.0;
        int r = lane;
        for (; r + 448 < rows; r += 512) {
            a0 += p[(size_t)r * stride];         a1 += p[(size_t)(r + 64) * stride];
            a2 += p[(size_t)(r + 128) * stride]; a3 += p[(size_t)(r + 192) * stride];
            a4 += p[(size_t)(r + 256) * stride]; a5 += p[(size_t)(r + 320) * stride];
            a6 += p[(size_t)(r + 384) * stride]; a7 += p[(size_t)(r + 448) * stride];
        }
        for (; r < rows; r += 64) a0 += p[(size_t)r * stride];
        return ((a0 + a1) + (a2 + a3)) + ((a4 + a5) + (a6 + a7));
    };
    double acc = 0.0;
    if (i < NL) {
        acc = colsum(pS + N + i / L, g.nch, ws);
    } else if (i < 2 * NL) {
        acc = colsum(pG + (i - NL), rowsG, NL);
    } else if (i < 3 * NL) {
        const int e = i - 2 * NL;
        if (e % L == 0) acc = colsum(pS + 2 * N + e / L, g.nch, ws);
    } else if (i < 3 * NL + N) {
        acc = colsum(pS + (i - 3 * NL), g.nch, ws);
    } else if (i < 3 * NL + N + 3) {
        acc = colsum(pS + 3 * N + (i - 3 * NL - N), g.nch, ws);
    }
    if (i < 3 * NL) {
        const int64_t T = g.T;
        const int pair = i % NL, which = i / NL, a = pair / L, k = pair % L + 1;
        const double *yc = y + (int64_t)ch * T, *rc = rho + (int64_t)ch * N * T;
        const double *yh = yhead + (int64_t)ch * (NL + 2);
        const double *V = virt + ((int64_t)ch * N + a) * (L + 1);
        const double z = Zc[(int64_t)ch * g.nch];
        if (g.first)
            for (int j = 1 + lane; j <= L - 1; j += 64) {
                const int idx = -j + k - 1;
                if (idx < 0) continue;
                const double rv = fexp((V[j] + yh[a * L + (L - 1 - j)]) - z);
                const double yv = yc[idx];
                acc += which == 0 ? rv : (which == 1 ? rv * yv : rv * (yv * yv));
            }
        if (which == 0) {
            if (g.last)
                for (int64_t t = T - L + 1 + lane; t <= T - k; t += 64)
                    if (t >= 0) acc += rc[(int64_t)a * T + t];
            if (lane == 0) {
                const double lpv = k == 1 ? Rf[((int64_t)ch * N + a) * T] : V[k - 1];
                pp[(int64_t)ch * S + 1 + pair] = (lpv + yh[a * L + (L - k)]) - z;
                if (pair == 0) pp[(int64_t)ch * S] = (FA0[(int64_t)ch * T] + yh[NL]) - z;
            }
        }
    }
    acc = wave_sum(acc);
    if (lane == 0) stats[(int64_t)ch * total + i] = acc;
}

__global__ __launch_bounds__(256) void kw_mstep(WaveGeom g, const WaveConst *__restrict__ cst,
                                                const double *__restrict__ stats_all,
                                                const double *__restrict__ pp_all, double *__restrict__ out_all)
{
    __shared__ double red[8];
    const int N = g.N, L = g.L, NL = N * L, K = L + 1, ch = blockIdx.x, S = 1 + NL;
    const double *stats = stats_all + (int64_t)ch * (3 * NL + N + 4);
    const double *pp = pp_all + (int64_t)ch * S;
    double *out = out_all + (int64_t)ch * (K * N + 1 + N + S);
    const double *G0 = stats, *G1 = stats + NL, *G2 = stats + 2 * NL, *Xi = stats + 3 * NL;
    const double s_all = stats[3 * NL + N], s_m = stats[3 * NL + N + 1], s_y2 = stats[3 * NL + N + 2];
    double x2 = 0.0, qq = 0.0;
    for (int p = threadIdx.x; p < NL; p += blockDim.x) {
        const int a = p / L, k = p % L + 1;
        const double mu = G1[p] / G0[p];
        out[k + K * a] = mu;
        x2 += (G2[p] - (2.0 * mu) * G1[p]) + (mu * mu) * G0[p];
        qq += G0[p];
    }
    for (int a = threadIdx.x; a < N; a += blockDim.x) {
        out[K * a] = 0.0;
        out[K * N + 1 + a] = (cst[ch].xishift[a] + flog(Xi[a])) - flog(s_m);
    }
    for (int j = threadIdx.x; j < S; j += blockDim.x) out[K * N + 1 + N + j] = pp[j];
    x2 = wave_sum(x2); qq = wave_sum(qq);
    if ((threadIdx.x & 63) == 0) { red[threadIdx.x >> 6] = x2; red[4 + (threadIdx.x >> 6)] = qq; }
    __syncthreads();
    if (threadIdx.x == 0) {
        const double X2 = ((red[0] + red[1]) + (red[2] + red[3])) + s_y2;
        const double QQ = ((red[4] + red[5]) + (red[6] + red[7])) + s_all;
        out[K * N] = sqrt(X2 / QQ);
    }
}

template <typename Kern>
static int wave_lds_attr2(Kern kern, size_t lds)
{
    if (lds > 64 * 1024)
        HS_HIP(hipFuncSetAttribute((const void *)kern, hipFuncAttributeMaxDynamicSharedMemorySize, (int)lds));
    return HMMSORT_OK;
}

static int wave_estep_sweeps(WaveDev *r, const double *d_y, double *d_stats, hipStream_t st, bool wait_cert = true)
{
    const WaveGeom &g = r->g;
    const int N = g.N, L = g.L, NL = N * L;
    const int nchT = g.C * g.nch;
    if (!r->keep_post) r->post_valid = false;
    int rowsG = 0;
    int rc = dispatch_N(N, [&](auto n) {
        constexpr int NN = decltype(n)::value;
        const size_t ldsf = ((size_t)(NN > 8 ? 1 : 2) * NN * (g.RB + 1) + 5 + 3 * NN + NN * NN) * sizeof(double);
        const bool generic = getenv("HMMSORT_GSUM_GENERIC") != nullptr;
        constexpr bool kFuse4 = NN == 3 || NN == 4, kFuse8 = NN >= 5 && NN <= 8;
        const bool sep = generic || r->keep_post || getenv("HMMSORT_GSUM_SEPARATE") != nullptr;
        const int ft = sep ? 0 : (kFuse4 && L <= 64) ? 1 : (kFuse8 && r->uniform_cx && L <= 64) ? 2
                       : (kFuse8 && r->uniform_cx && L <= 128) ? 4 : 0;
        const bool fuse = ft > 0;
        const int ym = bwd_yring(ft);
        const size_t ldsb = ((size_t)(NN + 1) * (g.RB + 1) + 4 + 3 * NN + NN * NN +
                             (fuse ? ym + (128 + 8 * (NN <= 4 ? 1 : 2)) * (NN <= 4 ? 4 : 8) : 0)) * sizeof(double);
        auto kf = kw_fwd<NN, true>;
        auto kb = kw_bwd<NN, true>;
        if constexpr (NN <= 8) {
            if (!r->uniform_cx) { kf = kw_fwd<NN, false>; kb = kw_bwd<NN, false>; }
        }
        if (r->keep_post) {
            kb = kw_bwd<NN, true, 0, true>;
            if constexpr (NN <= 8) {
                if (!r->uniform_cx) kb = kw_bwd<NN, false, 0, true>;
            }
        }
        if constexpr (kFuse4) {
            if (ft == 1) kb = r->uniform_cx ? kw_bwd<NN, true, 1> : kw_bwd<NN, false, 1>;
        }
        if constexpr (kFuse8) {
            if (ft == 2) kb = kw_bwd<NN, true, 2>;
            if (ft == 4) kb = kw_bwd<NN, true, 4>;
        }
        int rc2;
        if ((rc2 = wave_lds_attr2(kf, ldsf)) || (rc2 = wave_lds_attr2(kb, ldsb))) return rc2;
        { WPROF(r, "kw_fwd", st);
          hipLaunchKernelGGL(kf, dim3(nchT), dim3(64), ldsf, st, g, r->d_cst, d_y, r->Rf, r->virt, r->FA0,
                             r->FV, r->FREF, r->fpre, r->trash); }
        { WPROF(r, r->keep_post ? "kw_bwd_post" : "kw_bwd", st);
          hipLaunchKernelGGL(kb, dim3(nchT), dim3(64), ldsb, st, g, r->d_cst, d_y, r->Rf, r->FA0, r->FV,
                             r->FREF, r->fpre, r->W2, r->rho, r->partS, r->Zc, r->bpre, r->bown, r->yhead, r->trash, r->partG,
                             r->gsil); }
        HS_HIP(hipGetLastError());
        HS_HIP(hipEventRecord(r->ev_a, st));
        HS_HIP(hipStreamWaitEvent(r->side, r->ev_a, 0));
        if (g.nch > 1) {
            WPROF(r, "kw_fb_check", r->side);
            hipLaunchKernelGGL(kw_fb_check, dim3(nchT), dim3(64), 0, r->side, g, 1e-9, r->FA0, r->FV, r->FREF, r->fpre,
                               r->bpre, r->bown, r->rho, r->diag, r->dbg);
        }
        HS_HIP(hipEventRecord(r->ev_c, r->side));
        if (r->keep_post) return HMMSORT_OK;
        constexpr int NPx = NN <= 1 ? 1 : (NN <= 2 ? 2 : (NN <= 4 ? 4 : (NN <= 8 ? 8 : 16)));
        constexpr int LPTx = 16 * (16 / NPx), HSx = LPTx - 16;
        const int ntx = (L + LPTx - 1) / LPTx;
        if (fuse) {
            rowsG = g.nch;
        } else if (!generic) {
            static const int nt_big = getenv("HMMSORT_GSUM_TILES") ? atoi(getenv("HMMSORT_GSUM_TILES")) : 16;
            const int want = nt_big >= 16 ? 16 : (nt_big >= 8 ? 8 : 4);
            const int ntk = NN > 8 ? (ntx <= 4 ? 4 : (ntx <= 8 ? (want < 8 ? want : 8) : want)) : (ntx < 4 ? ntx : 4);
            const int ngrp = (ntx + ntk - 1) / ntk;
            rowsG = (int)((g.T + kGxSubs * 8 * (int64_t)kGxBv - 1) / (kGxSubs * 8 * (int64_t)kGxBv));
            constexpr int RRx = kGxTR + HSx, RRPx = RRx + RRx / 16 + 1;
            const size_t l1 = ((size_t)8 * (RRPx * NPx + 2) + (size_t)8 * (kGxTR + 19 + LPTx * (ntk - 1))) * 8;
            const size_t l2 = (size_t)4 * 4 * 64 * 8;
            const size_t lds = l1 > l2 ? l1 : l2;
            auto go = [&](auto kern) -> int {
                int rc3 = wave_lds_attr2(kern, lds);
                if (rc3) return rc3;
                WPROF(r, "kw_gsum", st);
                hipLaunchKernelGGL(kern, dim3(rowsG, g.C, ngrp), dim3(256), lds, st, g, d_y, r->rho, rowsG, r->partG);
                return HMMSORT_OK;
            };
            if constexpr (NN > 8) rc2 = ntk == 4 ? go(kw_gsum_mx<NN, 4>) : ntk == 8 ? go(kw_gsum_mx<NN, 8>) : go(kw_gsum_mx<NN, 16>);
            else rc2 = ntk == 1 ? go(kw_gsum_mx<NN, 1>) : ntk == 2 ? go(kw_gsum_mx<NN, 2>)
                       : ntk == 3 ? go(kw_gsum_mx<NN, 3>) : go(kw_gsum_mx<NN, 4>);
            if (rc2) return rc2;
        } else {
            rowsG = r->gparts;
            const size_t lds = ((size_t)NN * kGsSub + kGsSub + L) * sizeof(double);
            WPROF(r, "kw_gsum", st);
            hipLaunchKernelGGL(kw_gsum_generic, dim3(rowsG, g.C, (NL + 255) / 256), dim3(256), lds, st, g, d_y, r->rho, rowsG, r->partG);
        }
        HS_HIP(hipGetLastError());
        return HMMSORT_OK;
    });
    if (rc) return rc;
    if (r->keep_post) {
        HS_HIP(hipStreamWaitEvent(st, r->ev_c, 0));
        return HMMSORT_OK;
    }
    const int total = 3 * NL + N + 4;
    { WPROF(r, "kw_stats_final", st);
      hipLaunchKernelGGL(kw_stats_final, dim3(total, g.C), dim3(64), 0, st, g, rowsG, r->partG, r->partS, d_y, r->Rf,
                         r->virt, r->FA0, r->rho, r->Zc, r->yhead, r->pp, d_stats); }
    if (wait_cert) HS_HIP(hipStreamWaitEvent(st, r->ev_c, 0));
    HS_HIP(hipGetLastError());
    return HMMSORT_OK;
}

int wave_estep(WaveDev *r, const double *d_y, double *d_stats, hipStream_t st)
{
    r->post_valid = false;
    return wave_graphed(r, 2, d_y, d_stats, nullptr, nullptr, st, [&](hipStream_t s) -> int {
        int rc;
        HS_HIP(hipMemsetAsync(r->diag, 0, 8 * sizeof(int64_t), s));
        if ((rc = wave_prepare(r, d_y, s))) return rc;
        return wave_estep_sweeps(r, d_y, d_stats, s);
    });
}

int wave_post_sweeps(WaveDev *r, const double *d_y, hipStream_t st)
{
    int rc;
    HS_HIP(hipMemsetAsync(r->diag, 0, 8 * sizeof(int64_t), st));
    if ((rc = wave_prepare(r, d_y, st))) return rc;
    r->keep_post = true;
    rc = wave_estep_sweeps(r, d_y, nullptr, st);
    r->keep_post = false;
    return rc;
}

int wave_mstep(WaveDev *r, const double *d_stats, double *d_out, hipStream_t st)
{
    { WPROF(r, "kw_mstep", st);
      hipLaunchKernelGGL(kw_mstep, dim3(r->g.C), dim3(256), 0, st, r->g, r->d_cst, d_stats, r->pp, d_out); }
    HS_HIP(hipGetLastError());
    return HMMSORT_OK;
}

int wave_decode_estep(WaveDev *r, const double *d_y, int16_t *d_x, double *d_ll, double *d_stats, hipStream_t st)
{
    r->post_valid = false;
    return wave_graphed(r, 3, d_y, d_x, d_ll, d_stats, st, [&](hipStream_t s) -> int {
        int rc;
        HS_HIP(hipMemsetAsync(r->diag, 0, wave_zero_bytes(r, true), s));
        if ((rc = wave_prepare(r, d_y, s))) return rc;
        HS_HIP(hipEventRecord(r->ev_fork, s));
        HS_HIP(hipStreamWaitEvent(r->side2, r->ev_fork, 0));
        if ((rc = wave_estep_sweeps(r, d_y, d_stats, s, false))) return rc;
        if ((rc = wave_viterbi_sweep(r, d_y, r->side2))) return rc;
        const bool ll_trunk = r->g.C == 1 && r->g.N <= 4;
        if ((rc = wave_viterbi_post(r, d_y, d_x, d_ll, r->side2, true, ll_trunk, s))) return rc;
        if (!ll_trunk) {
            HS_HIP(hipEventRecord(r->ev_join, r->side2));
            HS_HIP(hipStreamWaitEvent(s, r->ev_join, 0));
        }
        HS_HIP(hipStreamWaitEvent(s, r->ev_c, 0));
        return HMMSORT_OK;
    });
}

}
```

### hmmspikesorter.jl_amd/csrc/wave_viterbi.hip

```cpp
#include <algorithm>
#include <cmath>
#include <type_traits>

#include "wave_common.h"

namespace hmmsort {

constexpr double kVitTol = 1e-9;

template <int N>
struct WIn {
    double y;
    double R[N];
};

template <int N, bool UC, bool redo>
__device__ __forceinline__ void vit_chain(const WaveGeom &g, const WaveConst *__restrict__ cst,
                                          const double *__restrict__ y, const double *__restrict__ Rf,
                                          const double *__restrict__ virt, const double *__restrict__ ysum,
                                          uint32_t *__restrict__ psi, double *__restrict__ vpre,
                                          double *__restrict__ vend, uint32_t *__restrict__ trash, const int cg)
{
    constexpr int EB = wpsi_bits_c(N), EPW = wpsi_epw_c(N), PW = wpsi_words_c(N), D = wave_depth<N>();
    constexpr int KC0 = 3, KCEND = 3 + N, KCXT = 3 + 2 * N, KSIZE = 3 + 2 * N + N * N;
    extern __shared__ double lds_vit[];
    double *KC = lds_vit;
    double *DL = lds_vit + KSIZE;
    const int lane = threadIdx.x;
    const int ch = cg / g.nch, c = cg % g.nch;
    const int L = g.L, W = g.W, RB = g.RB, B = g.B;
    const int64_t T = g.T;
    const int64_t tc = (int64_t)c * B;
    const int nc = (int)((T - tc) < B ? (T - tc) : B);
    const int64_t tend = tc + nc;
    const double *yc = y + (int64_t)ch * T;
    const double *Rc = Rf + (int64_t)ch * N * T;
    uint32_t *psic = psi + (int64_t)ch * T;
    const int64_t SR = 1 + N * L;
    const int64_t planePsi = (int64_t)g.C * T;
    const double thr = wave_thr(g, cst[ch], ysum, ch);

    for (int i = lane; i < N * (RB + 1); i += 64) DL[i] = -INFINITY;
    {
        const WaveConst &Kg = cst[ch];
        if (lane == 0) { KC[0] = Kg.c00; KC[1] = Kg.mean0; KC[2] = Kg.den; }
        if (lane < N) { KC[KC0 + lane] = Kg.c0[lane]; KC[KCEND + lane] = Kg.cend[lane]; }
        if (UC) { if (lane < N) KC[KCXT + lane] = Kg.cxin[lane]; }
        else for (int i = lane; i < N * N; i += 64) KC[KCXT + i] = Kg.cxT[i];
    }
    __syncthreads();
    int64_t tinit;
    double D0;
    if (redo) {
        tinit = tc - 1;
        D0 = vend[(cg - 1) * SR];
        for (int i = lane; i < N * L; i += 64) {
            const int a = i / L, j = i % L + 1;
            DL[a * (RB + 1) + (L + 1 - j)] = vend[(cg - 1) * SR + 1 + i];
        }
    } else if (c == 0) {
        tinit = 0;
        D0 = -cst[ch].A;
        for (int i = lane; i < N * L; i += 64) {
            const int a = i / L, j = i % L + 1;
            DL[a * (RB + 1) + (L - j)] = virt[((int64_t)ch * N + a) * (L + 1) + j];
        }
        if (lane < N) DL[lane * (RB + 1) + L] = Rc[(int64_t)lane * T];
    } else {
        tinit = tc - g.Hw;
        D0 = 0.0;
    }
    __syncthreads();

    const int n_total = (int)(tend - 1 - tinit);
    auto load = [&](WIn<N> &d, int off) {
        const int nact = n_total - off < W ? n_total - off : W;
        const int li = lane < nact ? lane : 0;
        int64_t tb = tinit + 1 + off;
        tb = tb < T ? tb : T - 1;
        d.y = (yc + tb)[li];
#pragma unroll
        for (int a = 0; a < N; a++) d.R[a] = (Rc + (int64_t)a * T + tb)[li];
    };
    int rs = (1 + lane) % RB, ws = (L + 1 + lane) % RB;
    auto run = [&](const WIn<N> &d, int off, auto store_tag) {
        constexpr int STORE = decltype(store_tag)::value;
        const int nact = n_total - off < W ? n_total - off : W;
        const bool live = lane < nact;
        const int64_t tb = tinit + 1 + off;
        double X[N];
#pragma unroll
        for (int a = 0; a < N; a++) {
            const double v = DL[a * (RB + 1) + rs];
            X[a] = live ? v : -INFINITY;
        }
        double e1 = -INFINITY, e2 = -INFINITY;
        int earg = 0;
#pragma unroll
        for (int a = 0; a < N; a++) {
            const double v = X[a] + KC[KCEND + a];
            earg = v > e1 ? a + 1 : earg;
            e2 = fmax(e2, fmin(e1, v));
            e1 = fmax(e1, v);
        }
        const double c00 = KC[0];
        const double dd = d.y - KC[1];
        const double q0 = -((dd * dd) / KC[2]);
        double sa = live ? c00 + q0 : 0.0;
        double sb = live ? e1 + q0 : -INFINITY;
        scan_maxplus(sa, sb);
        const double Dn = fmax(D0 + sa, sb);
        const double Dprev = lane_prev(Dn, D0);
        uint32_t pw[PW];
#pragma unroll
        for (int w = 0; w < PW; w++) pw[w] = 0u;
        {
            const double v0 = Dprev + c00;
            const bool ring = e1 > v0;
            const double gap = ring ? e1 - fmax(e2, v0) : v0 - e1;
            const uint32_t fl = gap < thr ? 1u : 0u;
            pw[0] = (ring ? (uint32_t)earg : 0u) | (fl << (EB - 1));
        }
        double m1 = -INFINITY, m2 = -INFINITY, m3 = -INFINITY;
        int i1 = 0, i2 = 0;
        if (UC) {
#pragma unroll
            for (int b = 0; b < N; b++) {
                const double v = X[b];
                const bool g1 = v > m1, g2 = v > m2;
                m3 = g2 ? m2 : fmax(m3, v);
                i2 = g1 ? i1 : (g2 ? b + 1 : i2);
                m2 = g1 ? m1 : (g2 ? v : m2);
                i1 = g1 ? b + 1 : i1;
                m1 = g1 ? v : m1;
            }
        }
        const int wsl = live ? ws : RB;
#pragma unroll
        for (int a = 0; a < N; a++) {
            double r1 = -INFINITY, r2 = -INFINITY;
            int rarg = 0;
            if (UC) {
                const double cin = KC[KCXT + a];
                const bool first = (a + 1 == i1), second = (a + 1 == i2);
                r1 = (first ? m2 : m1) + cin;
                rarg = first ? i2 : i1;
                r2 = ((first || second) ? m3 : m2) + cin;
                if (N == 1) { r1 = -INFINITY; r2 = -INFINITY; rarg = 0; }
            } else {
#pragma unroll
                for (int b = 0; b < N; b++) {
                    if (b == a) continue;
                    const double v = X[b] + KC[KCXT + a * N + b];
                    rarg = v > r1 ? b + 1 : rarg;
                    r2 = fmax(r2, fmin(r1, v));
                    r1 = fmax(r1, v);
                }
            }
            const double v0 = Dprev + KC[KC0 + a];
            const bool ring = r1 > v0;
            const double u = ring ? r1 : v0;
            const double gap = ring ? r1 - fmax(r2, v0) : v0 - r1;
            const uint32_t fl = gap < thr ? 1u : 0u;
            DL[a * (RB + 1) + wsl] = u + d.R[a];
            const uint32_t ent = (ring ? (uint32_t)rarg : 0u) | (fl << (EB - 1));
            pw[(a + 1) / EPW] |= ent << (((a + 1) % EPW) * EB);
            if (!UC) __builtin_amdgcn_sched_barrier(0);
        }
        if (STORE) {
#pragma unroll
            for (int w = 0; w < PW; w++) {
                uint32_t *dst = live ? psic + w * planePsi + tb + lane : trash + lane;
                *dst = pw[w];
            }
        }
        D0 = wave_bcast(Dn, nact - 1);
        rs += W; rs = rs >= RB ? rs - RB : rs;
        ws += W; ws = ws >= RB ? ws - RB : ws;
    };
    auto dump = [&](double *rec, int64_t tref) {
        __syncthreads();
        if (lane == 0) rec[0] = D0;
        for (int i = lane; i < N * L; i += 64) {
            const int a = i / L, j = i % L + 1;
            const int slot = (int)((tref - j - tinit + L) % RB);
            rec[1 + i] = DL[a * (RB + 1) + slot];
        }
        __syncthreads();
    };
    auto sweep = [&](int from, int to, auto store_tag) {
        WIn<N> buf[D];
#pragma unroll
        for (int i = 0; i < D; i++) load(buf[i], from + i * W);
        int off = from;
        for (; off + D * W <= to; off += D * W) {
#pragma unroll
            for (int i = 0; i < D; i++) {
                run(buf[i], off + i * W, store_tag);
                load(buf[i], off + (i + D) * W);
            }
        }
#pragma unroll
        for (int i = 0; i < D; i++)
            if (off + i * W < to) run(buf[i], off + i * W, store_tag);
    };
    const int n_warm = (redo || c == 0) ? 0 : g.Hw - 1;
    if (n_warm > 0) {
        sweep(0, n_warm, std::integral_constant<int, 0>());
        dump(vpre + cg * SR, tc);
    }
    sweep(n_warm, n_total, std::integral_constant<int, 1>());
    dump(vend + cg * SR, tend);
    if (redo) {
        for (int i = lane; i < SR; i += 64) vpre[cg * SR + i] = vend[(cg - 1) * SR + i];
    }
}

template <int N, bool UC>
__global__ __launch_bounds__(64, wave_occ<N>()) void kw_vit(WaveGeom g, const WaveConst *__restrict__ cst,
                                                            const double *__restrict__ y,
                                                            const double *__restrict__ Rf,
                                                            const double *__restrict__ virt,
                                                            const double *__restrict__ ysum,
                                                            uint32_t *__restrict__ psi, double *__restrict__ vpre,
                                                            double *__restrict__ vend, uint32_t *__restrict__ trash)
{
    vit_chain<N, UC, false>(g, cst, y, Rf, virt, ysum, psi, vpre, vend, trash, (int)blockIdx.x);
}

constexpr int kVitRedoGrid = 64;
template <int N, bool UC, bool TIGHT>
__global__ __launch_bounds__(64) __attribute__((amdgpu_waves_per_eu(TIGHT ? 6 : 1))) void kw_vit_redo(WaveGeom g, const WaveConst *__restrict__ cst,
                                                                 const double *__restrict__ y,
                                                                 const double *__restrict__ Rf,
                                                                 const double *__restrict__ virt,
                                                                 const double *__restrict__ ysum,
                                                                 uint32_t *__restrict__ psi, double *__restrict__ vpre,
                                                                 double *__restrict__ vend, uint32_t *__restrict__ trash,
                                                                 const int32_t *__restrict__ head,
                                                                 const int32_t *__restrict__ list)
{
    const int n = head[0];
    for (int q = blockIdx.x; q < n; q += gridDim.x)
        vit_chain<N, UC, true>(g, cst, y, Rf, virt, ysum, psi, vpre, vend, trash, list[q]);
}

struct VitCert {
    bool fail, anybad;
    double spread;
};

__device__ __forceinline__ VitCert vit_cert(const WaveGeom &g, const double *__restrict__ vpre,
                                            const double *__restrict__ vend, int cg, int lane, double *__restrict__ dbgrec)
{
    const int c = cg % g.nch;
    const int64_t SR = 1 + (int64_t)g.N * g.L;
    double lo = INFINITY, hi = -INFINITY;
    int64_t ilo = -1, ihi = -1, ibad = -1;
    bool bad = false;
    for (int64_t i = lane; i < SR; i += 64) {
        const double p = vpre[cg * SR + i], e = vend[(cg - 1) * SR + i];
        if (p == e) {
            if (fabs(p) < INFINITY) { lo = fmin(lo, 0.0); hi = fmax(hi, 0.0); }
            continue;
        }
        const double d = p - e;
        if (!(fabs(d) < INFINITY)) { bad = true; ibad = i; continue; }
        if (d < lo) { lo = d; ilo = i; }
        if (d > hi) { hi = d; ihi = i; }
    }
    if (dbgrec) {
        for (int o = 32; o > 0; o >>= 1) {
            const double l2 = __shfl_xor(lo, o), h2 = __shfl_xor(hi, o);
            const long long il2 = __shfl_xor((long long)ilo, o), ih2 = __shfl_xor((long long)ihi, o), ib2 = __shfl_xor((long long)ibad, o);
            if (l2 < lo) { lo = l2; ilo = il2; }
            if (h2 > hi) { hi = h2; ihi = ih2; }
            if (ib2 > ibad) ibad = ib2;
        }
        if (lane == 0 && c <= 3) {
            double *r = dbgrec + 16 + 8 * (c - 1);
            r[0] = (double)cg; r[1] = lo; r[2] = (double)ilo; r[3] = hi; r[4] = (double)ihi; r[5] = (double)ibad;
            r[6] = ilo >= 0 ? vpre[cg * SR + ilo] : 0.0; r[7] = ilo >= 0 ? vend[(cg - 1) * SR + ilo] : 0.0;
        }
    }
    lo = -wave_max(-lo); hi = wave_max(hi);
    VitCert v;
    v.anybad = __any(bad);
    v.spread = hi - lo;
    v.fail = v.anybad || !(v.spread <= kVitTol);
    return v;
}

__global__ __launch_bounds__(64) void kw_vit_check(WaveGeom g, const double *__restrict__ vpre,
                                                   const double *__restrict__ vend,
                                                   int32_t *__restrict__ vfail, int64_t *__restrict__ diag,
                                                   int final_round, double *__restrict__ dbg,
                                                   int32_t *__restrict__ head, int32_t *__restrict__ list)
{
    const int lane = threadIdx.x;
    const int cg = blockIdx.x, c = cg % g.nch;
    if (c == 0) { if (lane == 0) vfail[cg] = 0; return; }
    const VitCert v = vit_cert(g, vpre, vend, cg, lane, final_round ? dbg : nullptr);
    if (lane == 0) {
        vfail[cg] = v.fail ? 1 : 0;
        if (final_round) {
            if (v.fail) atomicAdd((unsigned long long *)&diag[0], 1ull);
            if (!v.anybad && v.spread == v.spread && v.spread < INFINITY) {
                const unsigned long long sb = (unsigned long long)__double_as_longlong(v.spread);
                if (sb > *reinterpret_cast<volatile unsigned long long *>(&diag[2]))
                    atomicMax((unsigned long long *)&diag[2], sb);
            }
        } else if (v.fail) {
            atomicAdd((unsigned long long *)&diag[1], 1ull);
        }
    }
    if (!final_round && v.fail) {
        const bool prev_fail = c > 1 && vit_cert(g, vpre, vend, cg - 1, lane, nullptr).fail;
        if (!prev_fail && lane == 0) list[atomicAdd(&head[0], 1)] = cg;
    }
}

__device__ __forceinline__ int vit_final_state(const WaveGeom &g, const WaveConst *__restrict__ cst,
                                               const double *__restrict__ ysum, const double *__restrict__ vend,
                                               int ch, int lane, bool *flagged)
{
    const int64_t SR = 1 + (int64_t)g.N * g.L;
    const double *rec = vend + ((int64_t)ch * g.nch + g.nch - 1) * SR;
    const int S = 1 + g.N * g.L;
    double best = -INFINITY, sec = -INFINITY;
    int bi = S;
    for (int j = lane; j < S; j += 64) {
        const double v = rec[j];
        if (v > best) { sec = best; best = v; bi = j; }
        else sec = fmax(sec, v);
    }
    for (int o = 32; o > 0; o >>= 1) {
        const double ov = __shfl_xor(best, o), os = __shfl_xor(sec, o);
        const int oi = __shfl_xor(bi, o);
        const bool take = ov > best || (ov == best && oi < bi);
        const double lose = take ? best : ov;
        sec = fmax(fmax(sec, os), lose);
        if (take) { best = ov; bi = oi; }
    }
    *flagged = (best - sec) < wave_thr(g, cst[ch], ysum, ch);
    return (bi >= S) ? 0 : bi;
}

template <int N>
__device__ __forceinline__ void bt_start(const WaveGeom &g, const WaveConst *__restrict__ cst,
                                         const double *__restrict__ ysum, const double *__restrict__ vend,
                                         int32_t *__restrict__ final_state, int64_t *__restrict__ tie_cnt, int ch, int lane,
                                         bool at_end, int &id, int &rem, int &wi, int &sh)
{
    constexpr int EB = wpsi_bits_c(N), EPW = wpsi_epw_c(N);
    if (!__any(at_end)) return;
    bool flagged;
    const int fs = vit_final_state(g, cst, ysum, vend, ch, lane, &flagged);
    if (blockIdx.x == gridDim.x - 1 && lane == 0) {
        final_state[ch] = fs;
        if (flagged) {
            tie_cnt[ch * 8 + kTieTail] = 1;
            atomicAdd((unsigned long long *)&tie_cnt[ch * 8 + kTieTrig], 1ull);
        }
    }
    if (at_end && fs > 0) {
        const int L = g.L, a0 = (fs - 1) / L, k0 = (fs - 1) % L + 1, e0 = a0 + 1;
        id = fs + 1; rem = k0 - 1; wi = e0 / EPW; sh = (e0 % EPW) * EB;
    }
}

template <int N> constexpr int bt_tile()
{
    constexpr int PW = wpsi_words_c(N);
    return PW == 1 ? 64 : (PW <= 3 ? 32 : 16);
}
template <int N> constexpr size_t bt_lds_bytes()
{
    constexpr int PW = wpsi_words_c(N), TS = bt_tile<N>();
    return sizeof(uint32_t) * (size_t)(PW * 64 * (TS + 4) + 64 * (TS / 2 + 1));
}

template <int N>
__device__ __forceinline__ void backtrace_light_body(const WaveGeom &g, const WaveConst *__restrict__ cst,
                                               const double *__restrict__ ysum, const double *__restrict__ vend,
                                               const uint32_t *__restrict__ psi, int32_t *__restrict__ final_state,
                                               int16_t *__restrict__ x, int32_t *__restrict__ bstate,
                                               int64_t *__restrict__ tie_cnt)
{
    constexpr int EB = wpsi_bits_c(N), EPW = wpsi_epw_c(N), PW = wpsi_words_c(N);
    constexpr int TS = bt_tile<N>();
    constexpr int RPI = 64 / TS;
    constexpr int XW = TS / 2;
    constexpr int XRI = 64 / XW;
    constexpr int CH = PW == 1 ? 8 : 4;
    constexpr int NCH = TS / CH;
    constexpr int TSP = TS + 4;
    constexpr int LPR = TS / 4;
    constexpr int RPW = 64 / LPR;
    constexpr int WU = 4;
    constexpr int SU = 2;
    constexpr int XU = PW == 4 ? 2 : 4;
    static_assert(CH % 4 == 0 && TS % CH == 0, "chunks are whole 16-byte groups");
    static_assert(64 % (RPW * WU) == 0, "whole batches of wide loads");
    static_assert(bt_lds_bytes<N>() <= 32 * 1024, "LDS budget");
    extern __shared__ __align__(16) uint32_t lds_bt[];
    uint32_t (*tile)[64][TSP] = reinterpret_cast<uint32_t (*)[64][TSP]>(lds_bt);
    uint32_t (*xt)[XW + 1] = reinterpret_cast<uint32_t (*)[XW + 1]>(lds_bt + PW * 64 * TSP);
    const int lane = threadIdx.x, ch = blockIdx.y;
    const int L = g.L, Bb = g.Bb, Hb = g.Hb;
    const int64_t T = g.T;
    const int64_t sg0 = (int64_t)blockIdx.x * 64, sg = sg0 + lane;
    const bool active = sg < g.nseg;
    const int64_t s_lo = sg * Bb;
    const int64_t s_hi = active ? ((s_lo + Bb) < T ? (s_lo + Bb) : T) : s_lo;
    const int64_t te = (s_hi + Hb) < T ? (s_hi + Hb) : T;
    const int64_t planePsi = (int64_t)g.C * T;
    const uint32_t *pc = psi + (int64_t)ch * T;
    int16_t *xc = x + (int64_t)ch * T;
    const bool xal = ((reinterpret_cast<uintptr_t>(xc)) & 3) == 0;
    const int te_rel = active ? (int)(te - s_lo) : 0, hi_rel = (int)(s_hi - s_lo);
    const int t1 = s_lo >= 1 ? 0 : 1;
    const int t2 = s_lo >= 2 ? 0 : (int)(2 - s_lo);
    int id = 1, rem = 0, wi = 0, sh = 0;
    bt_start<N>(g, cst, ysum, vend, final_state, tie_cnt, ch, lane, active && te == T, id, rem, wi, sh);
    int nflag = 0, bs = 0;
    const int lr = lane / TS, lc = lane % TS;
    auto walk = [&](int q, auto fast_tag, auto own_tag, bool emit) {
        constexpr bool FAST = decltype(fast_tag)::value, OWN = decltype(own_tag)::value;
#pragma unroll 1
        for (int k = NCH - 1; k >= 0; k--) {
            uint32_t rowv[PW][CH], xr[CH / 2];
#pragma unroll
            for (int w = 0; w < PW; w++)
#pragma unroll
                for (int i = 0; i < CH; i += 4) {
                    const uint4 t4 = *reinterpret_cast<const uint4 *>(&tile[w][lane][k * CH + i]);
                    rowv[w][i] = t4.x; rowv[w][i + 1] = t4.y; rowv[w][i + 2] = t4.z; rowv[w][i + 3] = t4.w;
                }
#pragma unroll
            for (int i = CH - 1; i >= 0; i--) {
                const int u = TS * q + k * CH + i;
                const bool interior = rem > 0;
                if (FAST ? OWN : true) {
                    if (i & 1) xr[i / 2] = (uint32_t)id << 16;
                    else xr[i / 2] |= (uint32_t)id & 0xffffu;
                }
                uint32_t wsel = rowv[0][i];
#pragma unroll
                for (int w = 1; w < PW; w++) wsel = (wi == w) ? rowv[w][i] : wsel;
                const uint32_t ent = wsel >> sh;
                const int pj = (int)(ent & ((1u << (EB - 1)) - 1u));
                const int flag = (int)((ent >> (EB - 1)) & 1u);
                const int jid = 1 + pj * L, jrem = pj ? L - 1 : 0;
                const int jwi = pj / EPW, jsh = (pj % EPW) * EB;
                if (FAST) {
                    if (OWN) nflag += interior ? 0 : flag;
                    id = interior ? id - 1 : jid;
                    rem = interior ? rem - 1 : jrem;
                    wi = interior ? wi : jwi;
                    sh = interior ? sh : jsh;
                } else {
                    const bool live = u < te_rel, step = live && u >= t1;
                    bs = (live && u == hi_rel) ? id : bs;
                    if (step && !interior && u < hi_rel && u >= t2) nflag += flag;
                    id = step ? (interior ? id - 1 : jid) : id;
                    rem = step ? (interior ? rem - 1 : jrem) : rem;
                    wi = step ? (interior ? wi : jwi) : wi;
                    sh = step ? (interior ? sh : jsh) : sh;
                }
            }
            if (FAST ? OWN : true) {
                if (emit) {
#pragma unroll
                    for (int j = 0; j < CH / 2; j++) xt[lane][k * (CH / 2) + j] = xr[j];
                }
            }
        }
    };
    const int nq = (Bb + Hb) / TS;
    for (int q = nq - 1; q >= 0; q--) {
        {
            const int64_t tb = sg0 * Bb + (int64_t)TS * q, left = T - tb;
            const int nrow = g.nseg - sg0 < 64 ? (int)(g.nseg - sg0) : 64;
            const int lim = left < 0 ? 0 : (left < (int64_t)64 * Bb ? (int)left : 64 * Bb);
#pragma unroll
            for (int w = 0; w < PW; w++) {
                const uint32_t *pw = pc + w * planePsi;
                if (T >= 4 && (reinterpret_cast<uintptr_t>(pw) & 15) == 0) {
                    const uint32_t *base = pw + (lim >= 4 ? tb : 0);
                    const int wr = lane / LPR, wc = 4 * (lane % LPR);
#pragma unroll 1
                    for (int r0 = 0; r0 < 64; r0 += RPW * WU) {
                        uint4 v[WU];
#pragma unroll
                        for (int j = 0; j < WU; j++) {
                            const int r = r0 + j * RPW + wr, o = r * Bb + wc;
                            const bool ok = r < nrow && o + 4 <= lim;
                            v[j] = *reinterpret_cast<const uint4 *>(base + (ok ? (uint32_t)o : 0u));
                        }
#pragma unroll
                        for (int j = 0; j < WU; j++) {
                            const int r = r0 + j * RPW + wr, o = r * Bb + wc;
                            const bool ok = r < nrow && o + 4 <= lim;
                            *reinterpret_cast<uint4 *>(&tile[w][r][wc]) = ok ? v[j] : make_uint4(0u, 0u, 0u, 0u);
                        }
                    }
                    if (left < (int64_t)64 * Bb && (lim & 3)) {
                        const int c0 = (lim & ~3) - lane * Bb;
                        if (c0 >= 0 && c0 < TS) {
#pragma unroll
                            for (int j = 0; j < 3; j++)
                                if (j < (lim & 3)) tile[w][lane][c0 + j] = pw[tb + (lim & ~3) + j];
                        }
                    }
                } else {
                    const uint32_t *base = pw + (lim > 0 ? tb : 0);
#pragma unroll SU
                    for (int rr = 0; rr < 64; rr += RPI) {
                        const int r = rr + lr, o = r * Bb + lc;
                        const bool ok = r < nrow && o < lim;
                        const uint32_t v = base[ok ? (uint32_t)o : 0u];
                        tile[w][r][lc] = ok ? v : 0u;
                    }
                }
            }
        }
        __syncthreads();
        const int u0 = TS * q, u1 = u0 + TS;
        const bool own_tile = u0 < Bb;
        const bool lane_fast = u0 >= t1 && u1 <= te_rel &&
                               (own_tile ? (u1 <= hi_rel && u0 >= t2) : (u0 > hi_rel));
        const bool fast = __all(lane_fast);
        if (fast && own_tile) walk(q, std::true_type(), std::true_type(), true);
        else if (fast) walk(q, std::true_type(), std::false_type(), false);
        else walk(q, std::false_type(), std::false_type(), own_tile);
        if (own_tile) {
            __syncthreads();
            const int xrw = lane / XW, xcw = lane % XW;
#pragma unroll XU
            for (int rr = 0; rr < 64; rr += XRI) {
                const int r = rr + xrw;
                const int64_t t = (sg0 + r) * Bb + (int64_t)TS * q + 2 * xcw;
                if ((sg0 + r) < g.nseg && t < T) {
                    const uint32_t v = xt[r][xcw];
                    if (t + 1 < T && xal) *reinterpret_cast<uint32_t *>(xc + t) = v;
                    else {
                        xc[t] = (int16_t)(v & 0xffffu);
                        if (t + 1 < T) xc[t + 1] = (int16_t)(v >> 16);
                    }
                }
            }
        }
        __syncthreads();
    }
    if (active && hi_rel < te_rel) (bstate + ((int64_t)ch * g.nseg + sg0))[lane] = bs;
    for (int o = 32; o > 0; o >>= 1) nflag += __shfl_xor(nflag, o);
    if (lane == 0 && nflag) atomicAdd((unsigned long long *)&tie_cnt[ch * 8 + kTieTrig], (unsigned long long)nflag);
}

template <int N>
__global__ __launch_bounds__(64) void kw_backtrace(WaveGeom g, const WaveConst *__restrict__ cst,
                                                   const double *__restrict__ ysum, const double *__restrict__ vend,
                                                   const uint32_t *__restrict__ psi, int32_t *__restrict__ final_state,
                                                   int16_t *__restrict__ x, int32_t *__restrict__ bstate,
                                                   int64_t *__restrict__ tie_cnt)
{
    constexpr int EB = wpsi_bits_c(N), EPW = wpsi_epw_c(N), PW = wpsi_words_c(N);
    constexpr int TS = PW <= 2 ? 64 : 32;
    constexpr int RPI = 64 / TS;
    constexpr int XW = TS / 2;
    constexpr int XRI = 64 / XW;
    __shared__ uint32_t tile[PW][64][TS + 1];
    __shared__ uint32_t xt[64][XW + 1];
    const int lane = threadIdx.x, ch = blockIdx.y;
    const int L = g.L, Bb = g.Bb, Hb = g.Hb;
    const int64_t T = g.T;
    const int64_t sg0 = (int64_t)blockIdx.x * 64, sg = sg0 + lane;
    const bool active = sg < g.nseg;
    const int64_t s_lo = sg * Bb;
    const int64_t s_hi = active ? ((s_lo + Bb) < T ? (s_lo + Bb) : T) : s_lo;
    const int64_t te = (s_hi + Hb) < T ? (s_hi + Hb) : T;
    const int64_t planePsi = (int64_t)g.C * T;
    const uint32_t *pc = psi + (int64_t)ch * T;
    int16_t *xc = x + (int64_t)ch * T;
    const bool xal = ((reinterpret_cast<uintptr_t>(xc)) & 3) == 0;
    const int te_rel = active ? (int)(te - s_lo) : 0, hi_rel = (int)(s_hi - s_lo);
    const int t1 = s_lo >= 1 ? 0 : 1;
    const int t2 = s_lo >= 2 ? 0 : (int)(2 - s_lo);
    int id = 1, rem = 0, wi = 0, sh = 0;
    bt_start<N>(g, cst, ysum, vend, final_state, tie_cnt, ch, lane, active && te == T, id, rem, wi, sh);
    int nflag = 0, bs = 0;
    const int lr = lane / TS, lc = lane % TS;
    constexpr bool ROWREG = PW <= 2;
    uint32_t rowv[ROWREG ? PW : 1][ROWREG ? TS : 1], xr[XW];
    auto walk = [&](int q, auto fast_tag, auto own_tag) {
        constexpr bool FAST = decltype(fast_tag)::value, OWN = decltype(own_tag)::value;
#pragma unroll
        for (int i = TS - 1; i >= 0; i--) {
            const int u = TS * q + i;
            const bool interior = rem > 0;
            if (FAST ? OWN : true) {
                if (i & 1) xr[i / 2] = (uint32_t)id << 16;
                else xr[i / 2] |= (uint32_t)id & 0xffffu;
            }
            uint32_t wsel;
            if constexpr (ROWREG) {
                wsel = rowv[0][i];
#pragma unroll
                for (int w = 1; w < PW; w++) wsel = (wi == w) ? rowv[w][i] : wsel;
            } else {
                wsel = tile[wi][lane][i];
            }
            const uint32_t ent = wsel >> sh;
            const int pj = (int)(ent & ((1u << (EB - 1)) - 1u));
            const int flag = (int)((ent >> (EB - 1)) & 1u);
            const int jid = 1 + pj * L, jrem = pj ? L - 1 : 0;
            const int jwi = pj / EPW, jsh = (pj % EPW) * EB;
            if (FAST) {
                if (OWN) nflag += interior ? 0 : flag;
                id = interior ? id - 1 : jid;
                rem = interior ? rem - 1 : jrem;
                wi = interior ? wi : jwi;
                sh = interior ? sh : jsh;
            } else {
                const bool live = u < te_rel, step = live && u >= t1;
                bs = (live && u == hi_rel) ? id : bs;
                if (step && !interior && u < hi_rel && u >= t2) nflag += flag;
                id = step ? (interior ? id - 1 : jid) : id;
                rem = step ? (interior ? rem - 1 : jrem) : rem;
                wi = step ? (interior ? wi : jwi) : wi;
                sh = step ? (interior ? sh : jsh) : sh;
            }
        }
    };
    const int nq = (Bb + Hb) / TS;
    for (int q = nq - 1; q >= 0; q--) {
        {
            const int64_t tb = sg0 * Bb + (int64_t)TS * q;
            const uint32_t *base = pc + (tb < T ? tb : 0);
#pragma unroll 16
            for (int rr = 0; rr < 64; rr += RPI) {
                const int r = rr + lr;
                const bool ok = (sg0 + r) < g.nseg && tb + (int64_t)r * Bb + lc < T;
                const uint32_t off = ok ? (uint32_t)(r * Bb + lc) : 0u;
                uint32_t v[PW];
#pragma unroll
                for (int w = 0; w < PW; w++) v[w] = (base + w * planePsi)[off];
#pragma unroll
                for (int w = 0; w < PW; w++) tile[w][r][lc] = ok ? v[w] : 0u;
            }
        }
        __syncthreads();
        if constexpr (ROWREG) {
#pragma unroll
            for (int w = 0; w < PW; w++)
#pragma unroll
                for (int i = 0; i < TS; i++) rowv[w][i] = tile[w][lane][i];
        }
        const int u0 = TS * q, u1 = u0 + TS;
        const bool own_tile = u0 < Bb;
        const bool lane_fast = u0 >= t1 && u1 <= te_rel &&
                               (own_tile ? (u1 <= hi_rel && u0 >= t2) : (u0 > hi_rel));
        const bool fast = __all(lane_fast);
        if (fast && own_tile) walk(q, std::true_type(), std::true_type());
        else if (fast) walk(q, std::true_type(), std::false_type());
        else walk(q, std::false_type(), std::false_type());
        if (own_tile) {
#pragma unroll
            for (int j = 0; j < XW; j++) xt[lane][j] = xr[j];
            __syncthreads();
            const int xrw = lane / XW, xcw = lane % XW;
#pragma unroll 8
            for (int rr = 0; rr < 64; rr += XRI) {
                const int r = rr + xrw;
                const int64_t t = (sg0 + r) * Bb + (int64_t)TS * q + 2 * xcw;
                if ((sg0 + r) < g.nseg && t < T) {
                    const uint32_t v = xt[r][xcw];
                    if (t + 1 < T && xal) *reinterpret_cast<uint32_t *>(xc + t) = v;
                    else {
                        xc[t] = (int16_t)(v & 0xffffu);
                        if (t + 1 < T) xc[t + 1] = (int16_t)(v >> 16);
                    }
                }
            }
        }
        __syncthreads();
    }
    if (active && hi_rel < te_rel) bstate[(int64_t)ch * g.nseg + sg] = bs;
    for (int o = 32; o > 0; o >>= 1) nflag += __shfl_xor(nflag, o);
    if (lane == 0 && nflag) atomicAdd((unsigned long long *)&tie_cnt[ch * 8 + kTieTrig], (unsigned long long)nflag);
}

template <int N>
__global__ __launch_bounds__(64) __attribute__((amdgpu_waves_per_eu(6)))
void kw_backtrace_light(WaveGeom g, const WaveConst *__restrict__ cst, const double *__restrict__ ysum,
                        const double *__restrict__ vend, const uint32_t *__restrict__ psi,
                        int32_t *__restrict__ final_state, int16_t *__restrict__ x, int32_t *__restrict__ bstate,
                        int64_t *__restrict__ tie_cnt)
{
    backtrace_light_body<N>(g, cst, ysum, vend, psi, final_state, x, bstate, tie_cnt);
}

__device__ __forceinline__ void wwalk_step(const WaveGeom &g, const uint32_t *__restrict__ pc, int64_t planePsi,
                                           int64_t t, int &a, int &k, int64_t &nflag)
{
    if (a >= 0 && k > 1) { k--; return; }
    const int e = a + 1;
    const uint32_t w = pc[(int64_t)(e / g.epw) * planePsi + t];
    const uint32_t ent = (w >> ((e % g.epw) * g.EB)) & ((1u << g.EB) - 1u);
    const int p = (int)(ent & ((1u << (g.EB - 1)) - 1u));
    if (t >= 2) nflag += ent >> (g.EB - 1);
    if (p == 0) { a = -1; k = 0; }
    else { a = p - 1; k = g.L; }
}

__device__ __forceinline__ void stitch_check_one(const WaveGeom &g, const int16_t *x, const int32_t *bstate,
                                                 int32_t *head, int32_t *list, int64_t i)
{
    const int ch = (int)(i / g.nseg);
    const int64_t sg = i % g.nseg;
    if (sg >= g.nseg - 1) return;
    if (bstate[i] != (int)x[(int64_t)ch * g.T + (sg + 1) * g.Bb]) list[atomicAdd(&head[0], 1)] = (int32_t)i;
}

__global__ void kw_stitch_check(WaveGeom g, const int16_t *__restrict__ x, const int32_t *__restrict__ bstate,
                                int32_t *__restrict__ head, int32_t *__restrict__ list)
{
    const int64_t i = (int64_t)blockIdx.x * blockDim.x + threadIdx.x;
    if (i >= (int64_t)g.C * g.nseg) return;
    stitch_check_one(g, x, bstate, head, list, i);
}

__global__ __launch_bounds__(64) void kw_stitch_fix_par(WaveGeom g, const uint32_t *__restrict__ psi,
                                                        int16_t *__restrict__ x, int32_t *__restrict__ bstate,
                                                        const int32_t *__restrict__ head,
                                                        const int32_t *__restrict__ redo, int64_t *__restrict__ diag,
                                                        int64_t *__restrict__ tie_cnt)
{
    extern __shared__ uint32_t shp[];
    const int lane = threadIdx.x, n = head[0];
    const int L = g.L, Bb = g.Bb, PW = g.PW;
    int16_t *xs = reinterpret_cast<int16_t *>(shp + (size_t)PW * (Bb + 1));
    const int64_t planePsi = (int64_t)g.C * g.T;
    for (int q = blockIdx.x; q < n; q += gridDim.x) {
        const int32_t id = redo[q];
        const int ch = (int)(id / g.nseg);
        const int64_t sg = id % g.nseg;
        bool succ = false;
        for (int j = lane; j < n; j += 64) succ = succ || (redo[j] == id + 1 && sg + 1 < g.nseg);
        if (__any(succ)) continue;
        const uint32_t *pc = psi + (int64_t)ch * g.T;
        int16_t *xc = x + (int64_t)ch * g.T;
        const int64_t lo = sg * Bb, tn = lo + Bb;
        const int want = xc[tn];
        if (bstate[(int64_t)ch * g.nseg + sg] == want) continue;
        for (int w = 0; w < PW; w++)
            for (int i = lane; i <= Bb; i += 64) shp[w * (Bb + 1) + i] = pc[w * planePsi + lo + i];
        __syncthreads();
        if (lane == 0) {
            int a = -1, k = 0;
            int64_t nflag = 0;
            if (want > 1) { a = (want - 2) / L; k = (want - 2) % L + 1; }
            auto step = [&](int i) {
                if (a >= 0 && k > 1) { k--; return; }
                const int e = a + 1;
                const uint32_t wv = shp[(e / g.epw) * (Bb + 1) + i];
                const uint32_t ent = (wv >> ((e % g.epw) * g.EB)) & ((1u << g.EB) - 1u);
                const int p = (int)(ent & ((1u << (g.EB - 1)) - 1u));
                if (lo + i >= 2) nflag += ent >> (g.EB - 1);
                if (p == 0) { a = -1; k = 0; }
                else { a = p - 1; k = L; }
            };
            step(Bb);
            for (int i = Bb - 1; i >= 0; i--) {
                xs[i] = (int16_t)((a < 0) ? 1 : 2 + a * L + (k - 1));
                if (lo + i == 0) break;
                if (i > 0) step(i);
            }
            bstate[(int64_t)ch * g.nseg + sg] = want;
            atomicAdd((unsigned long long *)&diag[1], 1ull);
            if (nflag) atomicAdd((unsigned long long *)&tie_cnt[ch * 8 + kTieTrig], (unsigned long long)nflag);
        }
        __syncthreads();
        for (int i = lane; i < Bb; i += 64) xc[lo + i] = xs[i];
        __syncthreads();
    }
}

__device__ __forceinline__ void first_state(const WaveGeom &g, const WaveConst *__restrict__ cst,
                                            const double *__restrict__ y, const double *__restrict__ mean,
                                            const double *__restrict__ ctab_all, int16_t *x, int ch)
{
    const int N = g.N, L = g.L, S = 1 + N * L;
    const double *ctab = ctab_all + (int64_t)ch * (1 + 2 * N + N * N + N * L);
    const double *c0 = ctab + 1, *cend = ctab + 1 + N, *cx = ctab + 1 + 2 * N, *cint = ctab + 1 + 2 * N + N * N;
    const double *mc = mean + (int64_t)ch * S;
    const double A = cst[ch].A, den = cst[ch].den;
    int16_t *xc = x + (int64_t)ch * g.T;
    const double y0 = y[(int64_t)ch * g.T];
    auto T1 = [&](int a, int k) {
        const double dd = y0 - mc[1 + a * L + (k - 1)];
        return A - (dd * dd) / den;
    };
    double best = -INFINITY;
    int arg = 1;
    auto cand = [&](int state, double t1, double lp) {
        const double tt = t1 + lp;
        if (tt > best) { best = tt; arg = state; }
    };
    const int x1 = *(const volatile int16_t *)&xc[1];
    if (x1 == 1) {
        cand(1, 0.0, ctab[0]);
        for (int a = 0; a < N; a++) cand(1 + a * L + L, T1(a, L), cend[a]);
    } else {
        const int b = (x1 - 2) / L, k = (x1 - 2) % L + 1;
        if (k == 1) {
            cand(1, 0.0, c0[b]);
            for (int a = 0; a < N; a++)
                if (a != b) cand(1 + a * L + L, T1(a, L), cx[a * N + b]);
        } else {
            cand(1 + b * L + (k - 1), T1(b, k - 1), cint[b * L + (k - 1)]);
        }
    }
    xc[0] = (int16_t)arg;
}

__global__ __launch_bounds__(256) void kw_stitch_fix(WaveGeom g, const WaveConst *__restrict__ cst,
                                                     const double *__restrict__ y, const double *__restrict__ mean,
                                                     const double *__restrict__ ctab_all,
                                                     const uint32_t *__restrict__ psi, int16_t *x, int32_t *bstate,
                                                     const int32_t *__restrict__ head1, int32_t *head2, int32_t *redo,
                                                     int64_t *__restrict__ diag, int64_t *__restrict__ tie_cnt)
{
    const int tid = threadIdx.x;
    if (head1[0] != 0) {
        const int64_t nsegT = (int64_t)g.C * g.nseg;
        for (int64_t i = tid; i < nsegT; i += blockDim.x) stitch_check_one(g, x, bstate, head2, redo, i);
        __threadfence();
        __syncthreads();
        if (tid == 0) {
            const int n = atomicAdd(&head2[0], 0);
            const volatile int32_t *lst = redo;
            const int L = g.L, Bb = g.Bb;
            const int64_t planePsi = (int64_t)g.C * g.T;
            int64_t fixes = 0;
            for (int q = 0; q < n; q++) {
                const int32_t ent = lst[q];
                const int ch = (int)(ent / g.nseg);
                int64_t nflag = 0;
                int64_t sg = ent % g.nseg;
                const uint32_t *pc = psi + (int64_t)ch * g.T;
                int16_t *xc = x + (int64_t)ch * g.T;
                while (sg >= 0) {
                    const int64_t tn = (sg + 1) * Bb;
                    const int want = xc[tn];
                    if (bstate[(int64_t)ch * g.nseg + sg] == want) break;
                    bstate[(int64_t)ch * g.nseg + sg] = want;
                    fixes++;
                    int a = -1, k = 0;
                    if (want > 1) { a = (want - 2) / L; k = (want - 2) % L + 1; }
                    wwalk_step(g, pc, planePsi, tn, a, k, nflag);
                    for (int64_t t = tn - 1; t >= sg * Bb; t--) {
                        xc[t] = (int16_t)((a < 0) ? 1 : 2 + a * L + (k - 1));
                        if (t == 0) break;
                        if (t > sg * Bb) wwalk_step(g, pc, planePsi, t, a, k, nflag);
                    }
                    sg--;
                }
                if (nflag) atomicAdd((unsigned long long *)&tie_cnt[ch * 8 + kTieTrig], (unsigned long long)nflag);
            }
            diag[1] += fixes;
        }
        __threadfence();
        __syncthreads();
    }
    if (g.T >= 2)
        for (int ch = tid; ch < g.C; ch += blockDim.x) first_state(g, cst, y, mean, ctab_all, x, ch);
}

__global__ __launch_bounds__(256) void kw_ll_partial(WaveGeom g, const WaveConst *__restrict__ cst,
                                                     const double *__restrict__ y, const int16_t *__restrict__ x,
                                                     const double *__restrict__ mean,
                                                     const double *__restrict__ ctab_all, double *__restrict__ part,
                                                     const int64_t *__restrict__ redo_cnt)
{
    __shared__ double red[4];
    const int ch = blockIdx.y, N = g.N, L = g.L, S = 1 + N * L;
    if (redo_cnt && redo_cnt[ch * 8 + kTieFlips] == 0) return;
    const int64_t T = g.T;
    const double *yc = y + (int64_t)ch * T, *mc = mean + (int64_t)ch * S;
    const int16_t *xc = x + (int64_t)ch * T;
    const double *ctab = ctab_all + (int64_t)ch * (1 + 2 * N + N * N + N * L);
    const double A = cst[ch].A, den = cst[ch].den;
    double acc = 0.0;
    for (int64_t u = (int64_t)blockIdx.x * blockDim.x + threadIdx.x + 1; u < T;
         u += (int64_t)gridDim.x * blockDim.x) {
        const int xp = xc[u - 1], xn = xc[u];
        const double d = yc[u] - mc[xn - 1];
        const double inc = wpath_lp(N, L, ctab, xp, xn) + (A - (d * d) / den);
        acc += (double)(T - u) * inc;
    }
    if (blockIdx.x == 0 && threadIdx.x == 0) {
        const int x0 = xc[0];
        if (x0 != 1) {
            const double d = yc[0] - mc[x0 - 1];
            acc += (double)(T - 1) * (A - (d * d) / den);
        }
    }
    acc = wave_sum(acc);
    if ((threadIdx.x & 63) == 0) red[threadIdx.x >> 6] = acc;
    __syncthreads();
    if (threadIdx.x == 0) part[(int64_t)ch * gridDim.x + blockIdx.x] = (red[0] + red[1]) + (red[2] + red[3]);
}

__global__ __launch_bounds__(256) void kw_sum_partials(const double *__restrict__ part, int n, double *__restrict__ out)
{
    __shared__ double red[4];
    const int ch = blockIdx.x;
    double acc = 0.0;
    for (int i = threadIdx.x; i < n; i += blockDim.x) acc += part[(int64_t)ch * n + i];
    acc = wave_sum(acc);
    if ((threadIdx.x & 63) == 0) red[threadIdx.x >> 6] = acc;
    __syncthreads();
    if (threadIdx.x == 0) out[ch] = (red[0] + red[1]) + (red[2] + red[3]);
}

template <typename Kern>
static int wave_lds_attr(Kern kern, size_t lds)
{
    if (lds > 64 * 1024)
        HS_HIP(hipFuncSetAttribute((const void *)kern, hipFuncAttributeMaxDynamicSharedMemorySize, (int)lds));
    return HMMSORT_OK;
}

constexpr int kVitRounds = 2;

int wave_viterbi_sweep(WaveDev *r, const double *d_y, hipStream_t st)
{
    const WaveGeom &g = r->g;
    const int nchT = g.C * g.nch;
    return dispatch_N(g.N, [&](auto n) {
        constexpr int N = decltype(n)::value;
        const size_t lds = ((size_t)N * (g.RB + 1) + 3 + 2 * N + N * N) * sizeof(double);
        auto kern = kw_vit<N, true>;
        if constexpr (N <= 8) { if (!r->uniform_cx) kern = kw_vit<N, false>; }
        int rc = wave_lds_attr(kern, lds);
        if (rc) return rc;
        { WPROF(r, "kw_vit", st);
          hipLaunchKernelGGL(kern, dim3(nchT), dim3(64), lds, st, g, r->d_cst, d_y, r->Rf, r->virt, r->ysum,
                             r->psi, r->vpre, r->vend, (uint32_t *)r->trash); }
        HS_HIP(hipGetLastError());
        return HMMSORT_OK;
    });
}

int wave_viterbi_post(WaveDev *r, const double *d_y, int16_t *d_x, double *d_ll, hipStream_t st, bool beside,
                      bool ll_beside, hipStream_t ll_st)
{
    const WaveGeom &g = r->g;
    const int nchT = g.C * g.nch;
    const bool light = g.backtrace == 2 || (g.backtrace == 0 && beside);
    int rc = dispatch_N(g.N, [&](auto n) {
        constexpr int N = decltype(n)::value;
        const size_t lds = ((size_t)N * (g.RB + 1) + 3 + 2 * N + N * N) * sizeof(double);
        auto kern = kw_vit_redo<N, true, false>;
        if constexpr (N <= 8) { if (!r->uniform_cx) kern = kw_vit_redo<N, false, false>; }
        if constexpr (N <= 4) { if (beside) kern = r->uniform_cx ? kw_vit_redo<N, true, true> : kw_vit_redo<N, false, true>; }
        int rc2 = wave_lds_attr(kern, lds);
        if (rc2) return rc2;
        for (int round = 0; round < kVitRounds && g.nch > 1; round++) {
            int32_t *head = r->heads + round, *list = r->vlist + (size_t)round * nchT;
            { WPROF(r, "kw_vit_check", st);
              hipLaunchKernelGGL(kw_vit_check, dim3(nchT), dim3(64), 0, st, g, r->vpre, r->vend, r->vfail, r->diag, 0, nullptr,
                                 head, list); }
            { WPROF(r, "kw_vit_redo", st);
              hipLaunchKernelGGL(kern, dim3(std::min(nchT, kVitRedoGrid)), dim3(64), lds, st, g, r->d_cst, d_y, r->Rf,
                                 r->virt, r->ysum, r->psi, r->vpre, r->vend, (uint32_t *)r->trash, head, list); }
        }
        { WPROF(r, "kw_vit_check", st);
          hipLaunchKernelGGL(kw_vit_check, dim3(nchT), dim3(64), 0, st, g, r->vpre, r->vend, r->vfail, r->diag, 1, r->dbg,
                             nullptr, nullptr); }
        { WPROF(r, "kw_backtrace", st);
          auto kb = light ? kw_backtrace_light<N> : kw_backtrace<N>;
          const size_t ldsb = light ? bt_lds_bytes<N>() : 0;
          hipLaunchKernelGGL(kb, dim3((unsigned)((g.nseg + 63) / 64), g.C), dim3(64), ldsb, st, g, r->d_cst, r->ysum, r->vend,
                             r->psi, r->final_state, d_x, r->bstate, r->tie_cnt); }
        HS_HIP(hipGetLastError());
        return HMMSORT_OK;
    });
    if (rc) return rc;
    const int64_t nsegT = (int64_t)g.C * g.nseg;
    { WPROF(r, "kw_stitch_check", st);
      hipLaunchKernelGGL(kw_stitch_check, dim3((unsigned)((nsegT + 255) / 256)), dim3(256), 0, st, g, d_x, r->bstate,
                         r->heads + 2, r->redo); }
    { WPROF(r, "kw_stitch_fix", st);
      const size_t ldsp = ((size_t)g.PW * (g.Bb + 1)) * sizeof(uint32_t) + (size_t)g.Bb * sizeof(int16_t) + 8;
      hipLaunchKernelGGL(kw_stitch_fix_par, dim3(256), dim3(64), ldsp, st, g, r->psi, d_x, r->bstate, r->heads + 2, r->redo,
                         r->diag, r->tie_cnt);
      hipLaunchKernelGGL(kw_stitch_fix, dim3(1), dim3(256), 0, st, g, r->d_cst, d_y, r->d_mean, r->d_ctab, r->psi, d_x,
                         r->bstate, r->heads + 2, r->heads + 3, r->redo + nsegT, r->diag, r->tie_cnt); }
    if (ll_beside) {
        HS_HIP(hipEventRecord(r->ev_x, st));
        HS_HIP(hipStreamWaitEvent(ll_st, r->ev_x, 0));
        WPROF(r, "kw_ll_partial", ll_st);
        hipLaunchKernelGGL(kw_ll_partial, dim3(r->nparts, g.C), dim3(256), 0, ll_st, g, r->d_cst, d_y, d_x, r->d_mean,
                           r->d_ctab, r->part, nullptr);
    }
    if ((rc = wave_tie_resolve(r, d_y, d_x, st))) return rc;
    if (!ll_beside) {
        ll_st = st;
        WPROF(r, "kw_ll_partial", st);
        hipLaunchKernelGGL(kw_ll_partial, dim3(r->nparts, g.C), dim3(256), 0, st, g, r->d_cst, d_y, d_x, r->d_mean,
                           r->d_ctab, r->part, nullptr);
    } else {
        HS_HIP(hipEventRecord(r->ev_b, st));
        HS_HIP(hipStreamWaitEvent(ll_st, r->ev_b, 0));
        WPROF(r, "kw_ll_redo", ll_st);
        hipLaunchKernelGGL(kw_ll_partial, dim3(r->nparts, g.C), dim3(256), 0, ll_st, g, r->d_cst, d_y, d_x, r->d_mean,
                           r->d_ctab, r->part, r->tie_cnt);
    }
    { WPROF(r, "kw_sum_partials", ll_st);
      hipLaunchKernelGGL(kw_sum_partials, dim3(g.C), dim3(256), 0, ll_st, r->part, r->nparts, d_ll); }
    HS_HIP(hipGetLastError());
    return HMMSORT_OK;
}

int wave_viterbi(WaveDev *r, const double *d_y, int16_t *d_x, double *d_ll, hipStream_t st)
{
    return wave_graphed(r, 1, d_y, d_x, d_ll, nullptr, st, [&](hipStream_t s) -> int {
        int rc;
        HS_HIP(hipMemsetAsync(r->diag, 0, wave_zero_bytes(r, true), s));
        if ((rc = wave_prepare(r, d_y, s))) return rc;
        if ((rc = wave_viterbi_sweep(r, d_y, s))) return rc;
        return wave_viterbi_post(r, d_y, d_x, d_ll, s, false, false, s);
    });
}

}
```

Baseline: 10490 Msamples/s.

## Skip redundant Viterbi certification rounds, halve backtrace segments per workgroup, drop LL side stream

kw_vit_check now returns early when the previous redo round found no failing chunks. It caches per-chunk spread certificates so the final round only reduces them, instead of recomputing every certificate. The light backtrace kernel is templated on segments per workgroup and uses 32 for single-word psi models, which gives more workgroups and smaller LDS tiles. The log-likelihood partial overlap on the trunk stream, with its conditional redo launch, is removed and serialized after tie resolution. The goal is to cut repeated check work and tune backtrace occupancy, at the cost of losing the LL overlap.

```diff
diff --git a/hmmspikesorter.jl_amd/csrc/capi.cpp b/hmmspikesorter.jl_amd/csrc/capi.cpp
--- a/hmmspikesorter.jl_amd/csrc/capi.cpp
+++ b/hmmspikesorter.jl_amd/csrc/capi.cpp
@@ -112,6 +112,9 @@
     } else if (!strcmp(key, "tie_debug")) {
         HS_CHECK(value >= 0 && value <= 3, HMMSORT_EINVAL, "set_option: tie_debug must be 0..3");
         options_modify([&](Options &o) { o.tie_debug = value; });
+    } else if (!strcmp(key, "cert_rounds")) {
+        HS_CHECK(value >= 0 && value <= 1, HMMSORT_EINVAL, "set_option: cert_rounds must be 0 or 1");
+        options_modify([&](Options &o) { o.cert_rounds = value; });
     } else if (!strcmp(key, "backtrace")) {
         HS_CHECK(value >= 0 && value <= 2, HMMSORT_EINVAL, "set_option: backtrace must be 0..2");
         options_modify([&](Options &o) { o.backtrace = value; });
@@ -142,6 +145,7 @@
     else if (!strcmp(key, "blocked_hbm_columns")) *value = o.blocked_hbm_columns;
     else if (!strcmp(key, "tie_scale")) *value = o.tie_scale;
     else if (!strcmp(key, "tie_debug")) *value = o.tie_debug;
+    else if (!strcmp(key, "cert_rounds")) *value = o.cert_rounds;
     else if (!strcmp(key, "backtrace")) *value = o.backtrace;
     else if (!strcmp(key, "fit_streams")) *value = o.fit_streams;
     else if (!strcmp(key, "last_escalations")) *value = last_escalations();
diff --git a/hmmspikesorter.jl_amd/csrc/hmmsort_internal.h b/hmmspikesorter.jl_amd/csrc/hmmsort_internal.h
--- a/hmmspikesorter.jl_amd/csrc/hmmsort_internal.h
+++ b/hmmspikesorter.jl_amd/csrc/hmmsort_internal.h
@@ -43,6 +43,7 @@
     int64_t blocked_hbm_columns = 0;
     int64_t tie_debug = 0;
     int64_t fit_streams = 4;
+    int64_t cert_rounds = 0;
     int64_t backtrace = 0;
 };
 Options options_get();
diff --git a/hmmspikesorter.jl_amd/csrc/wave_common.h b/hmmspikesorter.jl_amd/csrc/wave_common.h
--- a/hmmspikesorter.jl_amd/csrc/wave_common.h
+++ b/hmmspikesorter.jl_amd/csrc/wave_common.h
@@ -30,6 +30,7 @@
     int first, last;
     double thr_scale;
     int tie_debug;
+    int cert_rounds;
     int backtrace;
 };
 
@@ -52,7 +53,7 @@
     std::vector<char> ucx;
     const double *bound_y = nullptr;
     hipStream_t side = nullptr, side2 = nullptr;
-    hipEvent_t ev_fork = nullptr, ev_join = nullptr, ev_a = nullptr, ev_b = nullptr, ev_c = nullptr, ev_x = nullptr;
+    hipEvent_t ev_fork = nullptr, ev_join = nullptr, ev_a = nullptr, ev_c = nullptr;
     std::vector<ProfEntry> prof;
     int64_t S = 0, K = 0;
     std::vector<RingModel> ring;
@@ -72,6 +73,7 @@
     uint32_t *psi = nullptr;
     double *vpre = nullptr, *vend = nullptr;
     int32_t *vfail = nullptr;
+    uint64_t *vcert = nullptr;
     int32_t *bstate = nullptr;
     int32_t *redo = nullptr;
     int32_t *final_state = nullptr;
@@ -354,8 +356,7 @@
 int wave_profile_read(WaveDev *r, hipStream_t st, std::vector<std::string> &names,
                       std::vector<double> &ms, std::vector<int64_t> &calls);
 int wave_viterbi_sweep(WaveDev *r, const double *d_y, hipStream_t st);
-int wave_viterbi_post(WaveDev *r, const double *d_y, int16_t *d_x, double *d_ll, hipStream_t st, bool beside,
-                      bool ll_beside, hipStream_t ll_st);
+int wave_viterbi_post(WaveDev *r, const double *d_y, int16_t *d_x, double *d_ll, hipStream_t st, bool beside);
 int wave_viterbi(WaveDev *r, const double *d_y, int16_t *d_x, double *d_ll, hipStream_t st);
 int wave_tie_resolve(WaveDev *r, const double *d_y, int16_t *d_x, hipStream_t st);
 int wave_tie_stats(WaveDev *r, hipStream_t st, int64_t out[8]);
diff --git a/hmmspikesorter.jl_amd/csrc/wave_engine.hip b/hmmspikesorter.jl_amd/csrc/wave_engine.hip
--- a/hmmspikesorter.jl_amd/csrc/wave_engine.hip
+++ b/hmmspikesorter.jl_amd/csrc/wave_engine.hip
@@ -51,7 +51,7 @@
     g.T = T; g.C = C; g.N = N; g.L = L;
     g.own_lo = 0; g.own_hi = T; g.first = 1; g.last = 1;
     { const Options o = options_get(); g.thr_scale = (double)o.tie_scale; g.tie_debug = (int)o.tie_debug;
-      g.backtrace = (int)o.backtrace; }
+      g.backtrace = (int)o.backtrace; g.cert_rounds = (int)o.cert_rounds; }
     g.W = std::min(L, 64);
     g.RB = (int)wround_up(L + g.W, 32);
     int64_t H = halo_req > 0 ? halo_req : std::max<int64_t>(256, 4 * (int64_t)L);
@@ -229,6 +229,7 @@
     A(&r->vpre, nchT * (1 + N * L));
     A(&r->vend, nchT * (1 + N * L));
     A(&r->vfail, nchT + 8);
+    A(&r->vcert, nchT + 8);
     A(&r->bstate, C * g.nseg);
     A(&r->redo, 2 * C * g.nseg + 8);
     A(&r->vlist, 2 * nchT + 8);
@@ -300,9 +301,7 @@
         hipEventCreateWithFlags(&r->ev_fork, hipEventDisableTiming) != hipSuccess ||
         hipEventCreateWithFlags(&r->ev_join, hipEventDisableTiming) != hipSuccess ||
         hipEventCreateWithFlags(&r->ev_a, hipEventDisableTiming) != hipSuccess ||
-        hipEventCreateWithFlags(&r->ev_b, hipEventDisableTiming) != hipSuccess ||
-        hipEventCreateWithFlags(&r->ev_c, hipEventDisableTiming) != hipSuccess ||
-        hipEventCreateWithFlags(&r->ev_x, hipEventDisableTiming) != hipSuccess) {
+        hipEventCreateWithFlags(&r->ev_c, hipEventDisableTiming) != hipSuccess) {
         set_error("wave engine: could not create the internal stream/events");
         wave_destroy(r);
         return HMMSORT_EHIP;
@@ -315,7 +314,7 @@
 {
     if (!r) return;
     void *ptrs[] = {r->d_cst, r->d_mean, r->d_meanT, r->d_cint, r->d_msq, r->d_ctab, r->d_states, r->Rf, r->W2, r->virt, r->ysum,
-                    r->psi, r->vpre, r->vend, r->vfail, r->bstate, r->redo, r->final_state, r->part, r->FA0,
+                    r->psi, r->vpre, r->vend, r->vfail, r->vcert, r->bstate, r->redo, r->final_state, r->part, r->FA0,
                     r->FV, r->FREF, r->fpre, r->bpre, r->bown, r->rho, r->Zc, r->partS, r->partG, r->yhead,
                     r->extra, r->pp, r->diag, r->vlist, r->dbg, r->trash, r->tie_list, r->tie_off, r->tie_walk, r->tie_guess,
                     r->tie_c, r->tie_ok, r->tie_v, r->gsil, r->phead, r->plogz, r->pcnt};
@@ -324,9 +323,7 @@
     if (r->ev_fork) (void)hipEventDestroy(r->ev_fork);
     if (r->ev_join) (void)hipEventDestroy(r->ev_join);
     if (r->ev_a) (void)hipEventDestroy(r->ev_a);
-    if (r->ev_b) (void)hipEventDestroy(r->ev_b);
     if (r->ev_c) (void)hipEventDestroy(r->ev_c);
-    if (r->ev_x) (void)hipEventDestroy(r->ev_x);
     if (r->side) (void)hipStreamDestroy(r->side);
     if (r->side2) (void)hipStreamDestroy(r->side2);
     for (auto &e : r->prof) { (void)hipEventDestroy(e.a); (void)hipEventDestroy(e.b); }
diff --git a/hmmspikesorter.jl_amd/csrc/wave_estep.hip b/hmmspikesorter.jl_amd/csrc/wave_estep.hip
--- a/hmmspikesorter.jl_amd/csrc/wave_estep.hip
+++ b/hmmspikesorter.jl_amd/csrc/wave_estep.hip
@@ -1117,12 +1117,9 @@
         HS_HIP(hipStreamWaitEvent(r->side2, r->ev_fork, 0));
         if ((rc = wave_estep_sweeps(r, d_y, d_stats, s, false))) return rc;
         if ((rc = wave_viterbi_sweep(r, d_y, r->side2))) return rc;
-        const bool ll_trunk = r->g.C == 1 && r->g.N <= 4;
-        if ((rc = wave_viterbi_post(r, d_y, d_x, d_ll, r->side2, true, ll_trunk, s))) return rc;
-        if (!ll_trunk) {
-            HS_HIP(hipEventRecord(r->ev_join, r->side2));
-            HS_HIP(hipStreamWaitEvent(s, r->ev_join, 0));
-        }
+        if ((rc = wave_viterbi_post(r, d_y, d_x, d_ll, r->side2, true))) return rc;
+        HS_HIP(hipEventRecord(r->ev_join, r->side2));
+        HS_HIP(hipStreamWaitEvent(s, r->ev_join, 0));
         HS_HIP(hipStreamWaitEvent(s, r->ev_c, 0));
         return HMMSORT_OK;
     });
diff --git a/hmmspikesorter.jl_amd/csrc/wave_viterbi.hip b/hmmspikesorter.jl_amd/csrc/wave_viterbi.hip
--- a/hmmspikesorter.jl_amd/csrc/wave_viterbi.hip
+++ b/hmmspikesorter.jl_amd/csrc/wave_viterbi.hip
@@ -291,27 +291,55 @@
     return v;
 }
 
+constexpr unsigned long long kVitNoSpread = ~0ull;
+
+__device__ __forceinline__ void vit_spread_max(int64_t *__restrict__ diag, unsigned long long sb)
+{
+    if (sb > *reinterpret_cast<volatile unsigned long long *>(&diag[2]))
+        atomicMax((unsigned long long *)&diag[2], sb);
+}
+
 __global__ __launch_bounds__(64) void kw_vit_check(WaveGeom g, const double *__restrict__ vpre,
                                                    const double *__restrict__ vend,
                                                    int32_t *__restrict__ vfail, int64_t *__restrict__ diag,
                                                    int final_round, double *__restrict__ dbg,
-                                                   int32_t *__restrict__ head, int32_t *__restrict__ list)
+                                                   int32_t *__restrict__ head, int32_t *__restrict__ list,
+                                                   const int32_t *__restrict__ prev_head,
+                                                   unsigned long long *__restrict__ vcert)
 {
     const int lane = threadIdx.x;
     const int cg = blockIdx.x, c = cg % g.nch;
-    if (c == 0) { if (lane == 0) vfail[cg] = 0; return; }
+    const bool same = prev_head && prev_head[0] == 0;
+    if (same && !final_round) return;
+    if (c == 0 && !same) { if (lane == 0) vfail[cg] = 0; return; }
+    if (same) {
+        if (cg % 64 == 0) {
+            const int j = cg + lane;
+            unsigned long long sb = 0;
+            if (j < (int)gridDim.x && j % g.nch != 0) {
+                const unsigned long long v = vcert[j];
+                sb = v != kVitNoSpread ? v : 0;
+            }
+            for (int o = 32; o > 0; o >>= 1) {
+                const unsigned long long t = (unsigned long long)__shfl_xor((long long)sb, o);
+                sb = t > sb ? t : sb;
+            }
+            if (lane == 0 && sb) vit_spread_max(diag, sb);
+        }
+        if (c >= 1 && c <= 3) (void)vit_cert(g, vpre, vend, cg, lane, dbg);
+        return;
+    }
     const VitCert v = vit_cert(g, vpre, vend, cg, lane, final_round ? dbg : nullptr);
+    const bool counted = !v.anybad && v.spread == v.spread && v.spread < INFINITY;
+    const unsigned long long sb = (unsigned long long)__double_as_longlong(v.spread);
     if (lane == 0) {
         vfail[cg] = v.fail ? 1 : 0;
         if (final_round) {
             if (v.fail) atomicAdd((unsigned long long *)&diag[0], 1ull);
-            if (!v.anybad && v.spread == v.spread && v.spread < INFINITY) {
-                const unsigned long long sb = (unsigned long long)__double_as_longlong(v.spread);
-                if (sb > *reinterpret_cast<volatile unsigned long long *>(&diag[2]))
-                    atomicMax((unsigned long long *)&diag[2], sb);
-            }
-        } else if (v.fail) {
-            atomicAdd((unsigned long long *)&diag[1], 1ull);
+            if (counted) vit_spread_max(diag, sb);
+        } else {
+            vcert[cg] = counted ? sb : kVitNoSpread;
+            if (v.fail) atomicAdd((unsigned long long *)&diag[1], 1ull);
         }
     }
     if (!final_round && v.fail) {
@@ -374,13 +402,13 @@
     constexpr int PW = wpsi_words_c(N);
     return PW == 1 ? 64 : (PW <= 3 ? 32 : 16);
 }
-template <int N> constexpr size_t bt_lds_bytes()
+template <int N, int SPW> constexpr size_t bt_lds_bytes()
 {
     constexpr int PW = wpsi_words_c(N), TS = bt_tile<N>();
-    return sizeof(uint32_t) * (size_t)(PW * 64 * (TS + 4) + 64 * (TS / 2 + 1));
-}
-
-template <int N>
+    return sizeof(uint32_t) * (size_t)(PW * SPW * (TS + 4) + SPW * (TS / 2 + 1));
+}
+
+template <int N, int SPW>
 __device__ __forceinline__ void backtrace_light_body(const WaveGeom &g, const WaveConst *__restrict__ cst,
                                                const double *__restrict__ ysum, const double *__restrict__ vend,
                                                const uint32_t *__restrict__ psi, int32_t *__restrict__ final_state,
@@ -397,20 +425,23 @@
     constexpr int TSP = TS + 4;
     constexpr int LPR = TS / 4;
     constexpr int RPW = 64 / LPR;
-    constexpr int WU = 4;
+    constexpr int WU = SPW / RPW < 4 ? SPW / RPW : 4;
     constexpr int SU = 2;
     constexpr int XU = PW == 4 ? 2 : 4;
     static_assert(CH % 4 == 0 && TS % CH == 0, "chunks are whole 16-byte groups");
-    static_assert(64 % (RPW * WU) == 0, "whole batches of wide loads");
-    static_assert(bt_lds_bytes<N>() <= 32 * 1024, "LDS budget");
+    static_assert(SPW == 64 || SPW == 32 || SPW == 16, "segments per workgroup");
+    static_assert(WU >= 1 && SPW % (RPW * WU) == 0, "whole batches of wide loads");
+    static_assert(SPW % RPI == 0 && SPW % XRI == 0, "whole row instructions");
+    static_assert(bt_lds_bytes<N, SPW>() <= 32 * 1024, "LDS budget");
     extern __shared__ __align__(16) uint32_t lds_bt[];
-    uint32_t (*tile)[64][TSP] = reinterpret_cast<uint32_t (*)[64][TSP]>(lds_bt);
-    uint32_t (*xt)[XW + 1] = reinterpret_cast<uint32_t (*)[XW + 1]>(lds_bt + PW * 64 * TSP);
+    uint32_t (*tile)[SPW][TSP] = reinterpret_cast<uint32_t (*)[SPW][TSP]>(lds_bt);
+    uint32_t (*xt)[XW + 1] = reinterpret_cast<uint32_t (*)[XW + 1]>(lds_bt + PW * SPW * TSP);
     const int lane = threadIdx.x, ch = blockIdx.y;
     const int L = g.L, Bb = g.Bb, Hb = g.Hb;
     const int64_t T = g.T;
-    const int64_t sg0 = (int64_t)blockIdx.x * 64, sg = sg0 + lane;
-    const bool active = sg < g.nseg;
+    const int64_t sg0 = (int64_t)blockIdx.x * SPW, sg = sg0 + lane;
+    const bool walker = SPW == 64 || lane < SPW;
+    const bool active = walker && sg < g.nseg;
     const int64_t s_lo = sg * Bb;
     const int64_t s_hi = active ? ((s_lo + Bb) < T ? (s_lo + Bb) : T) : s_lo;
     const int64_t te = (s_hi + Hb) < T ? (s_hi + Hb) : T;
@@ -420,7 +451,7 @@
     const bool xal = ((reinterpret_cast<uintptr_t>(xc)) & 3) == 0;
     const int te_rel = active ? (int)(te - s_lo) : 0, hi_rel = (int)(s_hi - s_lo);
     const int t1 = s_lo >= 1 ? 0 : 1;
-    const int t2 = s_lo >= 2 ? 0 : (int)(2 - s_lo);
+    const int t2 = 2 * t1;
     int id = 1, rem = 0, wi = 0, sh = 0;
     bt_start<N>(g, cst, ysum, vend, final_state, tie_cnt, ch, lane, active && te == T, id, rem, wi, sh);
     int nflag = 0, bs = 0;
@@ -437,9 +468,10 @@
                     const uint4 t4 = *reinterpret_cast<const uint4 *>(&tile[w][lane][k * CH + i]);
                     rowv[w][i] = t4.x; rowv[w][i + 1] = t4.y; rowv[w][i + 2] = t4.z; rowv[w][i + 3] = t4.w;
                 }
+            const int ub = TS * q + k * CH;
+            const int te_c = te_rel - ub, hi_c = hi_rel - ub, t1_c = t1 - ub, t2_c = t1_c + t1;
 #pragma unroll
             for (int i = CH - 1; i >= 0; i--) {
-                const int u = TS * q + k * CH + i;
                 const bool interior = rem > 0;
                 if (FAST ? OWN : true) {
                     if (i & 1) xr[i / 2] = (uint32_t)id << 16;
@@ -460,9 +492,9 @@
                     wi = interior ? wi : jwi;
                     sh = interior ? sh : jsh;
                 } else {
-                    const bool live = u < te_rel, step = live && u >= t1;
-                    bs = (live && u == hi_rel) ? id : bs;
-                    if (step && !interior && u < hi_rel && u >= t2) nflag += flag;
+                    const bool live = i < te_c, step = live && i >= t1_c;
+                    bs = (live && i == hi_c) ? id : bs;
+                    if (step && !interior && i < hi_c && i >= t2_c) nflag += flag;
                     id = step ? (interior ? id - 1 : jid) : id;
                     rem = step ? (interior ? rem - 1 : jrem) : rem;
                     wi = step ? (interior ? wi : jwi) : wi;
@@ -479,10 +511,10 @@
     };
     const int nq = (Bb + Hb) / TS;
     for (int q = nq - 1; q >= 0; q--) {
+        const int64_t tb = sg0 * Bb + (int64_t)TS * q, left = T - tb;
+        const int nrow = g.nseg - sg0 < SPW ? (int)(g.nseg - sg0) : SPW;
+        const int lim = left < 0 ? 0 : (left < (int64_t)SPW * Bb ? (int)left : SPW * Bb);
         {
-            const int64_t tb = sg0 * Bb + (int64_t)TS * q, left = T - tb;
-            const int nrow = g.nseg - sg0 < 64 ? (int)(g.nseg - sg0) : 64;
-            const int lim = left < 0 ? 0 : (left < (int64_t)64 * Bb ? (int)left : 64 * Bb);
 #pragma unroll
             for (int w = 0; w < PW; w++) {
                 const uint32_t *pw = pc + w * planePsi;
@@ -490,7 +522,7 @@
                     const uint32_t *base = pw + (lim >= 4 ? tb : 0);
                     const int wr = lane / LPR, wc = 4 * (lane % LPR);
 #pragma unroll 1
-                    for (int r0 = 0; r0 < 64; r0 += RPW * WU) {
+                    for (int r0 = 0; r0 < SPW; r0 += RPW * WU) {
                         uint4 v[WU];
 #pragma unroll
                         for (int j = 0; j < WU; j++) {
@@ -505,9 +537,9 @@
                             *reinterpret_cast<uint4 *>(&tile[w][r][wc]) = ok ? v[j] : make_uint4(0u, 0u, 0u, 0u);
                         }
                     }
-                    if (left < (int64_t)64 * Bb && (lim & 3)) {
+                    if (left < (int64_t)SPW * Bb && (lim & 3)) {
                         const int c0 = (lim & ~3) - lane * Bb;
-                        if (c0 >= 0 && c0 < TS) {
+                        if (walker && c0 >= 0 && c0 < TS) {
 #pragma unroll
                             for (int j = 0; j < 3; j++)
                                 if (j < (lim & 3)) tile[w][lane][c0 + j] = pw[tb + (lim & ~3) + j];
@@ -516,7 +548,7 @@
                 } else {
                     const uint32_t *base = pw + (lim > 0 ? tb : 0);
 #pragma unroll SU
-                    for (int rr = 0; rr < 64; rr += RPI) {
+                    for (int rr = 0; rr < SPW; rr += RPI) {
                         const int r = rr + lr, o = r * Bb + lc;
                         const bool ok = r < nrow && o < lim;
                         const uint32_t v = base[ok ? (uint32_t)o : 0u];
@@ -530,32 +562,38 @@
         const bool own_tile = u0 < Bb;
         const bool lane_fast = u0 >= t1 && u1 <= te_rel &&
                                (own_tile ? (u1 <= hi_rel && u0 >= t2) : (u0 > hi_rel));
-        const bool fast = __all(lane_fast);
-        if (fast && own_tile) walk(q, std::true_type(), std::true_type(), true);
-        else if (fast) walk(q, std::true_type(), std::false_type(), false);
-        else walk(q, std::false_type(), std::false_type(), own_tile);
+        const bool fast = __all(lane_fast || !walker);
+        if (walker) {
+            if (fast && own_tile) walk(q, std::true_type(), std::true_type(), true);
+            else if (fast) walk(q, std::true_type(), std::false_type(), false);
+            else walk(q, std::false_type(), std::false_type(), own_tile);
+        }
         if (own_tile) {
             __syncthreads();
             const int xrw = lane / XW, xcw = lane % XW;
+            int16_t *xb = xc + (lim > 0 ? tb : 0);
 #pragma unroll XU
-            for (int rr = 0; rr < 64; rr += XRI) {
-                const int r = rr + xrw;
-                const int64_t t = (sg0 + r) * Bb + (int64_t)TS * q + 2 * xcw;
-                if ((sg0 + r) < g.nseg && t < T) {
+            for (int rr = 0; rr < SPW; rr += XRI) {
+                const int r = rr + xrw, o = r * Bb + 2 * xcw;
+                if (r < nrow && o < lim) {
                     const uint32_t v = xt[r][xcw];
-                    if (t + 1 < T && xal) *reinterpret_cast<uint32_t *>(xc + t) = v;
+                    if (o + 1 < lim && xal) *reinterpret_cast<uint32_t *>(xb + o) = v;
                     else {
-                        xc[t] = (int16_t)(v & 0xffffu);
-                        if (t + 1 < T) xc[t + 1] = (int16_t)(v >> 16);
+                        xb[o] = (int16_t)(v & 0xffffu);
+                        if (o + 1 < lim) xb[o + 1] = (int16_t)(v >> 16);
                     }
                 }
             }
         }
         __syncthreads();
     }
-    if (active && hi_rel < te_rel) (bstate + ((int64_t)ch * g.nseg + sg0))[lane] = bs;
+    {
+        const int64_t nb = g.nseg - 1 - sg0;
+        const int nbs = nb < SPW ? (int)nb : SPW;
+        if ((int)threadIdx.x < nbs) (bstate + ((int64_t)ch * g.nseg + sg0))[threadIdx.x] = bs;
+    }
     for (int o = 32; o > 0; o >>= 1) nflag += __shfl_xor(nflag, o);
-    if (lane == 0 && nflag) atomicAdd((unsigned long long *)&tie_cnt[ch * 8 + kTieTrig], (unsigned long long)nflag);
+    if (threadIdx.x == 0 && nflag) atomicAdd((unsigned long long *)&tie_cnt[ch * 8 + kTieTrig], (unsigned long long)nflag);
 }
 
 template <int N>
@@ -691,14 +729,14 @@
     if (lane == 0 && nflag) atomicAdd((unsigned long long *)&tie_cnt[ch * 8 + kTieTrig], (unsigned long long)nflag);
 }
 
-template <int N>
+template <int N, int SPW>
 __global__ __launch_bounds__(64) __attribute__((amdgpu_waves_per_eu(6)))
 void kw_backtrace_light(WaveGeom g, const WaveConst *__restrict__ cst, const double *__restrict__ ysum,
                         const double *__restrict__ vend, const uint32_t *__restrict__ psi,
                         int32_t *__restrict__ final_state, int16_t *__restrict__ x, int32_t *__restrict__ bstate,
                         int64_t *__restrict__ tie_cnt)
 {
-    backtrace_light_body<N>(g, cst, ysum, vend, psi, final_state, x, bstate, tie_cnt);
+    backtrace_light_body<N, SPW>(g, cst, ysum, vend, psi, final_state, x, bstate, tie_cnt);
 }
 
 __device__ __forceinline__ void wwalk_step(const WaveGeom &g, const uint32_t *__restrict__ pc, int64_t planePsi,
@@ -881,12 +919,10 @@
 __global__ __launch_bounds__(256) void kw_ll_partial(WaveGeom g, const WaveConst *__restrict__ cst,
                                                      const double *__restrict__ y, const int16_t *__restrict__ x,
                                                      const double *__restrict__ mean,
-                                                     const double *__restrict__ ctab_all, double *__restrict__ part,
-                                                     const int64_t *__restrict__ redo_cnt)
+                                                     const double *__restrict__ ctab_all, double *__restrict__ part)
 {
     __shared__ double red[4];
     const int ch = blockIdx.y, N = g.N, L = g.L, S = 1 + N * L;
-    if (redo_cnt && redo_cnt[ch * 8 + kTieFlips] == 0) return;
     const int64_t T = g.T;
     const double *yc = y + (int64_t)ch * T, *mc = mean + (int64_t)ch * S;
     const int16_t *xc = x + (int64_t)ch * T;
@@ -932,6 +968,8 @@
         HS_HIP(hipFuncSetAttribute((const void *)kern, hipFuncAttributeMaxDynamicSharedMemorySize, (int)lds));
     return HMMSORT_OK;
 }
+
+template <int N> constexpr int bt_spw() { return wpsi_words_c(N) == 1 ? 32 : 64; }
 
 constexpr int kVitRounds = 2;
 
@@ -954,8 +992,7 @@
     });
 }
 
-int wave_viterbi_post(WaveDev *r, const double *d_y, int16_t *d_x, double *d_ll, hipStream_t st, bool beside,
-                      bool ll_beside, hipStream_t ll_st)
+int wave_viterbi_post(WaveDev *r, const double *d_y, int16_t *d_x, double *d_ll, hipStream_t st, bool beside)
 {
     const WaveGeom &g = r->g;
     const int nchT = g.C * g.nch;
@@ -968,23 +1005,31 @@
         if constexpr (N <= 4) { if (beside) kern = r->uniform_cx ? kw_vit_redo<N, true, true> : kw_vit_redo<N, false, true>; }
         int rc2 = wave_lds_attr(kern, lds);
         if (rc2) return rc2;
+        auto prev_head = [&](int round) -> const int32_t * {
+            return (round > 0 && !g.cert_rounds && g.nch > 1) ? r->heads + round - 1 : nullptr;
+        };
         for (int round = 0; round < kVitRounds && g.nch > 1; round++) {
             int32_t *head = r->heads + round, *list = r->vlist + (size_t)round * nchT;
             { WPROF(r, "kw_vit_check", st);
               hipLaunchKernelGGL(kw_vit_check, dim3(nchT), dim3(64), 0, st, g, r->vpre, r->vend, r->vfail, r->diag, 0, nullptr,
-                                 head, list); }
+                                 head, list, prev_head(round), (unsigned long long *)r->vcert); }
             { WPROF(r, "kw_vit_redo", st);
               hipLaunchKernelGGL(kern, dim3(std::min(nchT, kVitRedoGrid)), dim3(64), lds, st, g, r->d_cst, d_y, r->Rf,
                                  r->virt, r->ysum, r->psi, r->vpre, r->vend, (uint32_t *)r->trash, head, list); }
         }
         { WPROF(r, "kw_vit_check", st);
           hipLaunchKernelGGL(kw_vit_check, dim3(nchT), dim3(64), 0, st, g, r->vpre, r->vend, r->vfail, r->diag, 1, r->dbg,
-                             nullptr, nullptr); }
+                             nullptr, nullptr, prev_head(kVitRounds), (unsigned long long *)r->vcert); }
         { WPROF(r, "kw_backtrace", st);
-          auto kb = light ? kw_backtrace_light<N> : kw_backtrace<N>;
-          const size_t ldsb = light ? bt_lds_bytes<N>() : 0;
-          hipLaunchKernelGGL(kb, dim3((unsigned)((g.nseg + 63) / 64), g.C), dim3(64), ldsb, st, g, r->d_cst, r->ysum, r->vend,
-                             r->psi, r->final_state, d_x, r->bstate, r->tie_cnt); }
+          const dim3 grid_rows((unsigned)((g.nseg + 63) / 64), g.C);
+          constexpr int SPW = bt_spw<N>();
+          if (!light)
+              hipLaunchKernelGGL(kw_backtrace<N>, grid_rows, dim3(64), 0, st, g, r->d_cst, r->ysum, r->vend, r->psi,
+                                 r->final_state, d_x, r->bstate, r->tie_cnt);
+          else
+              hipLaunchKernelGGL((kw_backtrace_light<N, SPW>), dim3((unsigned)((g.nseg + SPW - 1) / SPW), g.C), dim3(64),
+                                 (bt_lds_bytes<N, SPW>()), st, g, r->d_cst, r->ysum, r->vend, r->psi, r->final_state, d_x,
+                                 r->bstate, r->tie_cnt); }
         HS_HIP(hipGetLastError());
         return HMMSORT_OK;
     });
@@ -999,28 +1044,12 @@
                          r->diag, r->tie_cnt);
       hipLaunchKernelGGL(kw_stitch_fix, dim3(1), dim3(256), 0, st, g, r->d_cst, d_y, r->d_mean, r->d_ctab, r->psi, d_x,
                          r->bstate, r->heads + 2, r->heads + 3, r->redo + nsegT, r->diag, r->tie_cnt); }
-    if (ll_beside) {
-        HS_HIP(hipEventRecord(r->ev_x, st));
-        HS_HIP(hipStreamWaitEvent(ll_st, r->ev_x, 0));
-        WPROF(r, "kw_ll_partial", ll_st);
-        hipLaunchKernelGGL(kw_ll_partial, dim3(r->nparts, g.C), dim3(256), 0, ll_st, g, r->d_cst, d_y, d_x, r->d_mean,
-                           r->d_ctab, r->part, nullptr);
-    }
     if ((rc = wave_tie_resolve(r, d_y, d_x, st))) return rc;
-    if (!ll_beside) {
-        ll_st = st;
-        WPROF(r, "kw_ll_partial", st);
-        hipLaunchKernelGGL(kw_ll_partial, dim3(r->nparts, g.C), dim3(256), 0, st, g, r->d_cst, d_y, d_x, r->d_mean,
-                           r->d_ctab, r->part, nullptr);
-    } else {
-        HS_HIP(hipEventRecord(r->ev_b, st));
-        HS_HIP(hipStreamWaitEvent(ll_st, r->ev_b, 0));
-        WPROF(r, "kw_ll_redo", ll_st);
-        hipLaunchKernelGGL(kw_ll_partial, dim3(r->nparts, g.C), dim3(256), 0, ll_st, g, r->d_cst, d_y, d_x, r->d_mean,
-                           r->d_ctab, r->part, r->tie_cnt);
-    }
-    { WPROF(r, "kw_sum_partials", ll_st);
-      hipLaunchKernelGGL(kw_sum_partials, dim3(g.C), dim3(256), 0, ll_st, r->part, r->nparts, d_ll); }
+    { WPROF(r, "kw_ll_partial", st);
+      hipLaunchKernelGGL(kw_ll_partial, dim3(r->nparts, g.C), dim3(256), 0, st, g, r->d_cst, d_y, d_x, r->d_mean,
+                         r->d_ctab, r->part); }
+    { WPROF(r, "kw_sum_partials", st);
+      hipLaunchKernelGGL(kw_sum_partials, dim3(g.C), dim3(256), 0, st, r->part, r->nparts, d_ll); }
     HS_HIP(hipGetLastError());
     return HMMSORT_OK;
 }
@@ -1032,7 +1061,7 @@
         HS_HIP(hipMemsetAsync(r->diag, 0, wave_zero_bytes(r, true), s));
         if ((rc = wave_prepare(r, d_y, s))) return rc;
         if ((rc = wave_viterbi_sweep(r, d_y, s))) return rc;
-        return wave_viterbi_post(r, d_y, d_x, d_ll, s, false, false, s);
+        return wave_viterbi_post(r, d_y, d_x, d_ll, s, false);
     });
 }
 
```

Measured after the change: 10680 Msamples/s, median of 6. 1.9% higher.
